# ShinYwings/SingleHDR-tf2

Hardware: AMD Instinct MI355X
Metric: HDR images/sec (512x512) end-to-end inference, deq+lin+hal (higher is better)
Workload: dtype f32

## Files before the change

### include/shdr.h

```cpp
#ifndef SHDR_H_
#define SHDR_H_

#include <stdint.h>

#ifdef __cplusplus
extern "C" {
#endif

void shdr_config_reload(void);

#define SHDR_OK          0
#define SHDR_E_SHAPE    (-1)
#define SHDR_E_ALIGN    (-2)
#define SHDR_E_ARCH     (-3)
#define SHDR_E_LAUNCH   (-4)
#define SHDR_E_NULL     (-5)

#define SHDR_ACT_NONE   0
#define SHDR_ACT_RELU   1
#define SHDR_ACT_LRELU  2
#define SHDR_ACT_TANH   3

#define SHDR_ALGO_AUTO    0
#define SHDR_ALGO_MFMA    1
#define SHDR_ALGO_DIRECT  2
#define SHDR_ALGO_MFMA_REG 3
#define SHDR_ALGO_MFMA_F16  4
#define SHDR_ALGO_MFMA_BF16 5
#define SHDR_ALGO_AUTO_F16  6
#define SHDR_ALGO_AUTO_BF16 7
#define SHDR_ALGO_AUTO_EXACT 8

const char* shdr_last_error(void);
const char* shdr_version(void);

uint32_t shdr_crc32c(const void* data, uint64_t n, uint32_t crc);

int shdr_same_pad(int in_size, int k, int stride, int* out_size, int* pad_before);

typedef struct shdr_conv2d_desc {
  int32_t N, H, W;
  int32_t C1, C2;
  int32_t Cout, KH, KW;
  int32_t stride;
  int32_t pad_t, pad_l;
  int32_t Ho, Wo;
  float   x2_scale;
  int32_t act1, act2;
  int32_t res_cstride;
  int32_t y_cstride;
  int32_t algo;
  int32_t cout_valid;
  int64_t w_batch_stride;
  int32_t y_pix_stride, y_off_h, y_off_w, y_H, y_W;
  int32_t prologue;
  int32_t pool;
} shdr_conv2d_desc;
enum { SHDR_POOL_MAX = 0, SHDR_POOL_AVG = 1 };
enum { SHDR_PROLOGUE_NONE = 0, SHDR_PROLOGUE_BILINEAR2X = 1,
       SHDR_PROLOGUE_RANGE_SCALE = 2 };

int shdr_conv2d_fwd_f32(const shdr_conv2d_desc* d,
                        const float* x1, const float* x2, const float* w,
                        const float* bias, const float* scale, const float* shift,
                        const float* residual, float* y, void* stream);

int shdr_conv2d_fwd_yrange_f32(const shdr_conv2d_desc* d,
                               const float* x1, const float* x2, const float* w,
                               const float* bias, const float* scale, const float* shift,
                               const float* residual, float* y, float* y_range, void* stream);

enum {
  SHDR_PLAN_DIRECT = 0,
  SHDR_PLAN_MFMA = 1,
  SHDR_PLAN_WINOGRAD_FUSED = 2,
  SHDR_PLAN_WINOGRAD_PLANES = 3,
  SHDR_PLAN_X3 = 4,
  SHDR_PLAN_X3N = 5
};
int shdr_conv2d_plan_f32(const shdr_conv2d_desc* d, int has_residual);
int64_t shdr_conv2d_prepared_filter_elems_f32(const shdr_conv2d_desc* d, int has_residual);
int shdr_conv2d_filter_is_plain_f32(const shdr_conv2d_desc* d, int has_residual);
int shdr_conv2d_prepare_filter_f32(const shdr_conv2d_desc* d, int has_residual, const float* w, float* prepared, void* stream);
int64_t shdr_conv2d_workspace_bytes_f32(const shdr_conv2d_desc* d, int has_residual);
int shdr_conv2d_fwd_prepared_f32(const shdr_conv2d_desc* d, const float* x1, const float* x2, const float* prepared,
                                 const float* bias, const float* scale, const float* shift, const float* residual, float* y,
                                 float* y_pool, void* workspace, void* stream);
int shdr_conv2d_fwd_prepared_ranged_f32(const shdr_conv2d_desc* d, const float* x1, const float* x2, const float* prepared,
                                        const float* bias, const float* scale, const float* shift, const float* residual, float* y,
                                        float* y_pool, void* workspace, const float* x1_range, const float* x2_range, float* y_range,
                                        void* stream);
int shdr_conv2d_projected_ok_f32(const shdr_conv2d_desc* d);
int shdr_conv2d_fwd_prepared_projected_f32(const shdr_conv2d_desc* d, const float* x1, const float* x2, const float* prepared,
                                           const float* bias, const float* scale, const float* shift, const float* proj, float* y_proj,
                                           float* y, float* y_pool, void* workspace, const float* x1_range, const float* x2_range,
                                           float* y_range, void* stream);

int shdr_conv2d_up2_lowres_ok_f32(const shdr_conv2d_desc* d);
int64_t shdr_conv2d_up2_lowres_filter_elems_f32(const shdr_conv2d_desc* d);
int shdr_conv2d_up2_lowres_prepare_filter_f32(const shdr_conv2d_desc* d, const float* w, float* prepared, void* stream);
int64_t shdr_conv2d_up2_lowres_workspace_bytes_f32(const shdr_conv2d_desc* d);
int shdr_conv2d_fwd_up2_lowres_f32(const shdr_conv2d_desc* d, const float* x, const float* prepared, const float* bias,
                                   const float* scale, const float* shift, float* y, void* workspace, const float* x_range,
                                   float* y_range, void* stream);

int shdr_conv2d_up2_fused_ok_f32(const shdr_conv2d_desc* d);
int shdr_conv2d_up2_narrow_enabled(void);
int64_t shdr_conv2d_up2_fused_filter_elems_f32(const shdr_conv2d_desc* d);
int shdr_conv2d_up2_fused_prepare_filter_f32(const shdr_conv2d_desc* d, const float* w, float* prepared, void* stream);
int shdr_conv2d_fwd_up2_fused_f32(const shdr_conv2d_desc* d, const float* x, const float* prepared, const float* bias,
                                  const float* scale, const float* shift, const float* proj, float* y_proj, float* y,
                                  const float* x_range, float* y_range, void* stream);

int shdr_conv2d_wgrad_f32(const shdr_conv2d_desc* d, const float* x, int which, const float* dz,
                          float* dw, void* stream);
int shdr_filter_transform_f32(const float* w, float* wt, int KH, int KW, int Cin, int Cout,
                              int c_begin, int c_count, float scale, void* stream);
int64_t shdr_conv2d_dgrad_workspace_bytes_f32(const shdr_conv2d_desc* d, int which);
int shdr_conv2d_dgrad_f32(const shdr_conv2d_desc* d, int which, const float* dz, const float* w, float* dx, void* workspace,
                          void* stream);
int shdr_conv2d_dgrad_tracks_range_f32(const shdr_conv2d_desc* d, int which);
int shdr_conv2d_dgrad_ranged_f32(const shdr_conv2d_desc* d, int which, const float* dz, const float* w, float* dx, void* workspace,
                                 const float* dz_range, float* dx_range, void* stream);
enum { SHDR_OP_CONV2D_FWD = 0, SHDR_OP_CONV2D_DGRAD = 1, SHDR_OP_CONV2D_WGRAD_WINOGRAD = 2, SHDR_OP_BATCHNORM = 3,
       SHDR_OP_ACT_BWD_BIAS = 4  };
#define SHDR_BN_MAX_BLOCKS 1024
int64_t shdr_workspace_bytes(int op, const shdr_conv2d_desc* d, int arg);
int shdr_bias_grad_f32(const float* dz, float* db, int64_t npix, int C, void* stream);

int shdr_soft_hist_fwd_f32(const float* x, float* y, int64_t npix, int C, int B, void* stream);
int shdr_soft_hist_bwd_f32(const float* x, const float* dy, float* dx, int64_t npix, int C, int B, void* stream);

int shdr_lin_frontend_fwd_f32(const float* img, float* y, int N, int H, int W,
                              int y_channels, void* stream);

int shdr_avgpool2_fwd_f32(const float* x, float* y, int N, int H, int W, int C, void* stream);
int shdr_maxpool2_fwd_f32(const float* x, float* y, int N, int H, int W, int C, void* stream);
int shdr_maxpool3s2_fwd_f32(const float* x, float* y, int N, int H, int W, int C, void* stream);
int shdr_resize2x_fwd_f32(const float* x, float* y, int N, int H, int W, int C, void* stream);
int shdr_gap_fwd_f32(const float* x, float* y, int N, int HW, int C, void* stream);

int shdr_invcrf_decode_fwd_f32(const float* feat, const float* wfc, const float* bfc,
                               const float* table, float* out, int B, int F, int K,
                               void* stream);
int shdr_increase_fwd_f32(const float* rf, float* out, int B, int K, void* stream);
int shdr_apply_rf_fwd_f32(const float* x, const float* rf, float* y, int B,
                          int64_t n_per_batch, int K, void* stream);

int shdr_clip_fwd_f32(const float* x, float* y, int64_t n, float lo, float hi, void* stream);
int shdr_vgg_preprocess_fwd_f32(const float* x, float* y, int64_t npix, int out_channels,
                                void* stream);
int shdr_reverse3_fwd_f32(const float* x, float* y, int64_t npix, void* stream);
int shdr_alpha_blend_fwd_f32(const float* b, const float* hal, float* a, float* alpha_out,
                             int64_t npix, float thr, void* stream);
int shdr_pack3_fwd_f32(const float* s0, const float* s1, const float* s2, const float* s3,
                       int nsrc, float* y, int out_channels, int64_t npix, void* stream);
int shdr_pad_channels_f32(const float* x, float* y, int64_t npix, int Cin, int Cout, void* stream);
// ... 389 lines not shown
```

### singlehdr-tf2_amd/_lib.py

```python
import ctypes
import os

_HERE = os.path.dirname(os.path.abspath(__file__))
LIB_PATH = os.environ.get("SHDR_LIB") or os.path.join(_HERE, "libshdr.so")

c_int = ctypes.c_int
c_i64 = ctypes.c_int64
c_f32 = ctypes.c_float
c_ptr = ctypes.c_void_p


class ConvDesc(ctypes.Structure):
    _fields_ = [("N", ctypes.c_int32), ("H", ctypes.c_int32), ("W", ctypes.c_int32),
                ("C1", ctypes.c_int32), ("C2", ctypes.c_int32),
                ("Cout", ctypes.c_int32), ("KH", ctypes.c_int32), ("KW", ctypes.c_int32),
                ("stride", ctypes.c_int32), ("pad_t", ctypes.c_int32), ("pad_l", ctypes.c_int32),
                ("Ho", ctypes.c_int32), ("Wo", ctypes.c_int32),
                ("x2_scale", ctypes.c_float),
                ("act1", ctypes.c_int32), ("act2", ctypes.c_int32),
                ("res_cstride", ctypes.c_int32), ("y_cstride", ctypes.c_int32),
                ("algo", ctypes.c_int32), ("cout_valid", ctypes.c_int32),
                ("w_batch_stride", ctypes.c_int64),
                ("y_pix_stride", ctypes.c_int32), ("y_off_h", ctypes.c_int32), ("y_off_w", ctypes.c_int32),
                ("y_H", ctypes.c_int32), ("y_W", ctypes.c_int32),
# ... 9 lines not shown
    "shdr_resize_cubic_f32": (c_int, [c_ptr, c_ptr, c_int, c_int, c_int, c_int, c_int, c_int, c_ptr]),
    "shdr_pad_symmetric_f32": (c_int, [c_ptr, c_ptr, c_int, c_int, c_int, c_int, c_int, c_ptr]),
    "shdr_rgbe_encode_f32": (c_int, [c_ptr, c_ptr, c_i64, c_int, c_ptr]),
    "shdr_rgbe_rle_encode": (c_i64, [c_ptr, c_int, c_int, c_ptr, c_i64]),
    "shdr_rgbe_rle_decode": (c_i64, [c_ptr, c_i64, c_int, c_int, c_ptr]),
    "shdr_rgbe_rle_encode_batch_sizes": (c_int, [c_ptr, c_int, ctypes.POINTER(c_i64), ctypes.POINTER(c_i64)]),
    "shdr_rgbe_rle_encode_batch": (c_int, [c_ptr, c_ptr, c_ptr, c_int, c_ptr, c_i64, c_ptr, c_ptr, c_ptr]),
    "shdr_rgbe_rle_encode_batch_timed": (c_int, [c_ptr, c_ptr, c_ptr, c_int, c_ptr, c_i64, c_ptr, c_ptr, c_ptr, c_ptr]),
    "shdr_hdr_load_resize_f32": (c_int, [c_ptr, c_ptr, c_int, c_int, c_int, c_int, c_ptr]),
    "shdr_hdr_window_means_f32": (c_int, [c_ptr, c_ptr, c_ptr, c_int, c_ptr, c_ptr, c_ptr]),
    "shdr_hdr_patch_sample_f32": (c_int, [c_ptr] * 5 + [c_int] * 4 + [c_ptr, c_ptr]),
    "shdr_exr_rle_decode": (c_i64, [c_ptr, c_i64, c_ptr, c_i64]),
    "shdr_exr_unpredict_u8": (c_int, [c_ptr, c_ptr, c_i64, c_ptr, c_ptr, c_int, c_ptr]),
    "shdr_exr_load_resize_f32": (c_int, [c_ptr, c_i64, c_ptr, c_int, c_int, c_i64, c_ptr, c_ptr, c_int, c_int, c_ptr, c_int, c_int,
                                         c_int, c_ptr]),
    "shdr_deflate_huffman_host": (c_i64, [c_ptr, c_i64, c_ptr, c_i64]),
    "shdr_deflate_huffman_lengths_host": (c_int, [c_ptr, c_i64, c_ptr]),
    "shdr_deflate_huffman_batch_sizes": (c_int, [c_ptr, c_int, c_int, ctypes.POINTER(c_i64), ctypes.POINTER(c_i64)]),
    "shdr_deflate_huffman_batch": (c_int, [c_ptr, c_ptr, c_ptr, c_ptr, c_int, c_int, c_ptr, c_i64, c_ptr, c_ptr, c_ptr, c_ptr, c_ptr]),
    "shdr_deflate_lz_host": (c_i64, [c_ptr, c_i64, c_ptr, c_i64]),
    "shdr_deflate_lz_parse_host": (c_int, [c_ptr, c_i64, c_ptr]),
    "shdr_deflate_lz_batch_sizes": (c_int, [c_ptr, c_int, c_int, ctypes.POINTER(c_i64), ctypes.POINTER(c_i64)]),
    "shdr_deflate_lz_batch": (c_int, [c_ptr, c_ptr, c_ptr, c_ptr, c_int, c_int, c_ptr, c_i64, c_ptr, c_ptr, c_ptr, c_ptr, c_ptr]),
    "shdr_inflate_host": (c_i64, [c_ptr, c_i64, c_ptr, c_i64, ctypes.POINTER(c_int)]),
    "shdr_inflate_batch_sizes": (c_int, [c_ptr, c_ptr, c_int, ctypes.POINTER(c_i64), ctypes.POINTER(c_i64)]),
    "shdr_piz_decode_host": (c_i64, [c_ptr, c_i64, c_int, c_int, c_ptr, c_int, c_ptr, c_i64, ctypes.POINTER(c_int)]),
    "shdr_piz_batch_sizes": (c_int, [c_ptr, c_ptr, c_ptr, c_ptr, c_int, c_int, c_int] + [ctypes.POINTER(c_i64)] * 3),
    "shdr_piz_batch": (c_int, [c_ptr, c_i64, c_ptr, c_ptr, c_ptr, c_i64, c_ptr, c_ptr, c_ptr, c_ptr, c_ptr, c_ptr, c_ptr, c_int, c_int, c_int,
                               c_ptr, c_i64, c_ptr, c_ptr, c_ptr, c_ptr, c_ptr]),
    "shdr_inflate_batch": (c_int, [c_ptr, c_i64, c_ptr, c_ptr, c_ptr, c_i64, c_ptr, c_ptr, c_ptr, c_int, c_ptr, c_ptr, c_ptr, c_ptr]),
    "shdr_exr_pack_sizes": (c_int, [c_ptr, c_int, c_int, c_int, ctypes.POINTER(c_i64), ctypes.POINTER(c_i64), c_ptr, c_ptr]),
    "shdr_exr_pack_f32": (c_int, [c_ptr, c_ptr, c_int, c_int, c_int, c_int, c_int, c_ptr, c_ptr, c_ptr, c_ptr, c_ptr]),
    "shdr_exr_finish_chunks": (c_int, [c_ptr, c_ptr, c_ptr, c_ptr, c_ptr, c_int, c_i64, c_int, c_ptr]),
    "shdr_philox4x32_10": (c_int, [c_ptr, c_ptr, c_ptr]),
    "shdr_camera_expose_f32": (c_int, [c_ptr, c_ptr, c_ptr, c_ptr, c_int, c_int, c_int, ctypes.c_uint64, c_ptr]),
    "shdr_jpeg_round_trip_f32": (c_int, [c_ptr] * 6 + [c_int, c_int, c_int, c_ptr]),
    "shdr_flip_rot90_f32": (c_int, [c_ptr, c_ptr, c_ptr, c_ptr, c_int, c_int, c_int, c_f32, c_ptr]),
    "shdr_pair_patch_stats": (c_int, [c_ptr, c_ptr, c_i64, c_ptr, c_ptr, c_int, c_ptr, c_ptr, c_int, c_int, c_ptr, c_ptr, c_ptr]),
    "shdr_pair_patch_gather_f32": (c_int, [c_ptr, c_ptr, c_i64, c_ptr, c_ptr, c_int, c_ptr, c_ptr, c_int, c_ptr, c_ptr, c_ptr, c_int,
                                           c_int, c_ptr, c_ptr, c_ptr]),
    "shdr_conv2d_winograd_fused_f32": (c_int, [c_ptr] * 6 + [c_int] * 7 + [c_ptr]),
    "shdr_conv2d_winograd_fused2_f32": (c_int, [c_ptr] * 8 + [c_int] * 8 + [c_ptr]),
    "shdr_conv2d_winograd_fused_up2_f32": (c_int, [c_ptr] * 6 + [c_int] * 7 + [c_ptr]),
    "shdr_conv2d_x3_ok_f32": (c_int, [ctypes.POINTER(ConvDesc)]),
    "shdr_conv2d_x3_filter_elems_f32": (c_i64, [ctypes.POINTER(ConvDesc)]),
    "shdr_conv2d_x3_prepare_filter_f32": (c_int, [ctypes.POINTER(ConvDesc), c_ptr, c_ptr, c_ptr]),
    "shdr_conv2d_fwd_x3_f32": (c_int, [ctypes.POINTER(ConvDesc)] + [c_ptr] * 9),
    "shdr_conv2d_fwd_x3_ranged_f32": (c_int, [ctypes.POINTER(ConvDesc)] + [c_ptr] * 12),
    "shdr_absmax_f32": (c_int, [c_ptr, c_i64, c_ptr, c_ptr]),
    "shdr_x3_split_planes_f32": (c_int, [c_ptr, c_i64, c_ptr, c_ptr, c_ptr, c_ptr]),
    "shdr_conv2d_wgrad_x3_ok_f32": (c_int, [ctypes.POINTER(ConvDesc), c_int]),
    "shdr_conv2d_wgrad_x3_f32": (c_int, [ctypes.POINTER(ConvDesc), c_ptr, c_ptr, c_int, c_ptr, c_ptr, c_ptr, c_ptr, c_ptr, c_ptr]),
    "shdr_config_reload": (None, []),
    "shdr_conv2d_x3_input_absmax_f32": (c_int, [c_ptr, c_i64, c_ptr, c_ptr]),
    "shdr_conv2d_x3n_ok_f32": (c_int, [ctypes.POINTER(ConvDesc)]),
    "shdr_conv2d_x3n_filter_elems_f32": (c_i64, [ctypes.POINTER(ConvDesc)]),
    "shdr_conv2d_x3n_prepare_filter_f32": (c_int, [ctypes.POINTER(ConvDesc), c_ptr, c_ptr, c_ptr]),
    "shdr_conv2d_fwd_x3n_f32": (c_int, [ctypes.POINTER(ConvDesc)] + [c_ptr] * 10),
    "shdr_conv2d_fwd_x3n_ranged_f32": (c_int, [ctypes.POINTER(ConvDesc)] + [c_ptr] * 13),
    "shdr_act_bwd_bias_f32": (c_int, [c_ptr, c_ptr, c_ptr, c_ptr, c_ptr, c_i64, c_int, c_int, c_ptr]),
    "shdr_winograd_filter_packed_f32": (c_int, [c_ptr, c_ptr, c_int, c_int, c_ptr]),
    "shdr_conv2d_wgrad_winograd_f32": (c_int, [c_ptr] * 4 + [c_int] * 7 + [c_f32, c_ptr]),
    "shdr_crc32c": (ctypes.c_uint32, [c_ptr, ctypes.c_uint64, ctypes.c_uint32]),
    "shdr_same_pad": (c_int, [c_int, c_int, c_int, ctypes.POINTER(c_int), ctypes.POINTER(c_int)]),
    "shdr_conv2d_fwd_f32": (c_int, [ctypes.POINTER(ConvDesc)] + [c_ptr] * 9),
    "shdr_conv2d_fwd_yrange_f32": (c_int, [ctypes.POINTER(ConvDesc)] + [c_ptr] * 10),
    "shdr_conv2d_plan_f32": (c_int, [ctypes.POINTER(ConvDesc), c_int]),
    "shdr_conv2d_prepared_filter_elems_f32": (c_i64, [ctypes.POINTER(ConvDesc), c_int]),
    "shdr_conv2d_filter_is_plain_f32": (c_int, [ctypes.POINTER(ConvDesc), c_int]),
    "shdr_conv2d_prepare_filter_f32": (c_int, [ctypes.POINTER(ConvDesc), c_int, c_ptr, c_ptr, c_ptr]),
    "shdr_conv2d_workspace_bytes_f32": (c_i64, [ctypes.POINTER(ConvDesc), c_int]),
    "shdr_conv2d_fwd_prepared_f32": (c_int, [ctypes.POINTER(ConvDesc)] + [c_ptr] * 11),
    "shdr_conv2d_fwd_prepared_ranged_f32": (c_int, [ctypes.POINTER(ConvDesc)] + [c_ptr] * 14),
    "shdr_conv2d_projected_ok_f32": (c_int, [ctypes.POINTER(ConvDesc)]),
    "shdr_conv2d_fwd_prepared_projected_f32": (c_int, [ctypes.POINTER(ConvDesc)] + [c_ptr] * 15),
    "shdr_conv2d_up2_lowres_ok_f32": (c_int, [ctypes.POINTER(ConvDesc)]),
    "shdr_conv2d_up2_lowres_filter_elems_f32": (c_i64, [ctypes.POINTER(ConvDesc)]),
    "shdr_conv2d_up2_lowres_prepare_filter_f32": (c_int, [ctypes.POINTER(ConvDesc), c_ptr, c_ptr, c_ptr]),
    "shdr_conv2d_up2_lowres_workspace_bytes_f32": (c_i64, [ctypes.POINTER(ConvDesc)]),
    "shdr_conv2d_fwd_up2_lowres_f32": (c_int, [ctypes.POINTER(ConvDesc)] + [c_ptr] * 10),
    "shdr_conv2d_up2_fused_ok_f32": (c_int, [ctypes.POINTER(ConvDesc)]),
    "shdr_conv2d_up2_narrow_enabled": (c_int, []),
    "shdr_conv2d_up2_fused_filter_elems_f32": (c_i64, [ctypes.POINTER(ConvDesc)]),
    "shdr_conv2d_up2_fused_prepare_filter_f32": (c_int, [ctypes.POINTER(ConvDesc), c_ptr, c_ptr, c_ptr]),
    "shdr_conv2d_fwd_up2_fused_f32": (c_int, [ctypes.POINTER(ConvDesc)] + [c_ptr] * 11),
    "shdr_conv2d_fwd_x3_projected_f32": (c_int, [ctypes.POINTER(ConvDesc)] + [c_ptr] * 14),
    "shdr_conv2d_fwd_x3_residual_f32": (c_int, [ctypes.POINTER(ConvDesc)] + [c_ptr] * 12),
    "shdr_conv2d_dgrad_workspace_bytes_f32": (c_i64, [ctypes.POINTER(ConvDesc), c_int]),
    "shdr_conv2d_dgrad_f32": (c_int, [ctypes.POINTER(ConvDesc), c_int, c_ptr, c_ptr, c_ptr, c_ptr, c_ptr]),
    "shdr_conv2d_dgrad_tracks_range_f32": (c_int, [ctypes.POINTER(ConvDesc), c_int]),
    "shdr_conv2d_dgrad_ranged_f32": (c_int, [ctypes.POINTER(ConvDesc), c_int, c_ptr, c_ptr, c_ptr, c_ptr, c_ptr, c_ptr, c_ptr]),
    "shdr_workspace_bytes": (c_i64, [c_int, ctypes.POINTER(ConvDesc), c_int]),
    "shdr_soft_hist_bwd_f32": (c_int, [c_ptr, c_ptr, c_ptr, c_i64, c_int, c_int, c_ptr]),
    "shdr_conv2d_wgrad_f32": (c_int, [ctypes.POINTER(ConvDesc), c_ptr, c_int, c_ptr, c_ptr, c_ptr]),
    "shdr_filter_transform_f32": (c_int, [c_ptr, c_ptr, c_int, c_int, c_int, c_int, c_int, c_int, c_f32, c_ptr]),
    "shdr_bias_grad_f32": (c_int, [c_ptr, c_ptr, c_i64, c_int, c_ptr]),
    "shdr_soft_hist_fwd_f32": (c_int, [c_ptr, c_ptr, c_i64, c_int, c_int, c_ptr]),
    "shdr_lin_frontend_fwd_f32": (c_int, [c_ptr, c_ptr, c_int, c_int, c_int, c_int, c_ptr]),
    "shdr_avgpool2_fwd_f32": (c_int, [c_ptr, c_ptr, c_int, c_int, c_int, c_int, c_ptr]),
    "shdr_maxpool2_fwd_f32": (c_int, [c_ptr, c_ptr, c_int, c_int, c_int, c_int, c_ptr]),
    "shdr_maxpool3s2_fwd_f32": (c_int, [c_ptr, c_ptr, c_int, c_int, c_int, c_int, c_ptr]),
    "shdr_resize2x_fwd_f32": (c_int, [c_ptr, c_ptr, c_int, c_int, c_int, c_int, c_ptr]),
    "shdr_gap_fwd_f32": (c_int, [c_ptr, c_ptr, c_int, c_int, c_int, c_ptr]),
    "shdr_invcrf_decode_fwd_f32": (c_int, [c_ptr] * 5 + [c_int, c_int, c_int, c_ptr]),
    "shdr_increase_fwd_f32": (c_int, [c_ptr, c_ptr, c_int, c_int, c_ptr]),
    "shdr_apply_rf_fwd_f32": (c_int, [c_ptr, c_ptr, c_ptr, c_int, c_i64, c_int, c_ptr]),
    "shdr_clip_fwd_f32": (c_int, [c_ptr, c_ptr, c_i64, c_f32, c_f32, c_ptr]),
    "shdr_vgg_preprocess_fwd_f32": (c_int, [c_ptr, c_ptr, c_i64, c_int, c_ptr]),
    "shdr_reverse3_fwd_f32": (c_int, [c_ptr, c_ptr, c_i64, c_ptr]),
    "shdr_alpha_blend_fwd_f32": (c_int, [c_ptr, c_ptr, c_ptr, c_ptr, c_i64, c_f32, c_ptr]),
    "shdr_pack3_fwd_f32": (c_int, [c_ptr] * 4 + [c_int, c_ptr, c_int, c_i64, c_ptr]),
    "shdr_logc_fwd_f32": (c_int, [c_ptr, c_ptr, c_i64, c_ptr]),
    "shdr_affine_act_f32": (c_int, [c_ptr] * 5 + [c_i64, c_int, c_int, c_ptr]),
    "shdr_pad_channels_f32": (c_int, [c_ptr, c_ptr, c_i64, c_int, c_int, c_ptr]),
    "shdr_act_bwd_f32": (c_int, [c_ptr, c_ptr, c_ptr, c_i64, c_int, c_ptr]),
    "shdr_clip_bwd_f32": (c_int, [c_ptr, c_ptr, c_ptr, c_i64, c_f32, c_f32, c_ptr]),
    "shdr_add_f32": (c_int, [c_ptr, c_ptr, c_ptr, c_i64, c_ptr]),
    "shdr_add_ranged_f32": (c_int, [c_ptr, c_ptr, c_ptr, c_i64, c_ptr, c_ptr]),
    "shdr_avgpool2_bwd_f32": (c_int, [c_ptr, c_ptr, c_int, c_int, c_int, c_int, c_ptr]),
    "shdr_maxpool2_bwd_f32": (c_int, [c_ptr, c_ptr, c_ptr, c_int, c_int, c_int, c_int, c_ptr]),
    "shdr_maxpool3s2_bwd_f32": (c_int, [c_ptr, c_ptr, c_ptr, c_ptr, c_int, c_int, c_int, c_int, c_ptr]),
    "shdr_resize2x_bwd_f32": (c_int, [c_ptr, c_ptr, c_int, c_int, c_int, c_int, c_ptr]),
    "shdr_resize2x_bwd_ranged_f32": (c_int, [c_ptr, c_ptr, c_int, c_int, c_int, c_int, c_ptr, c_ptr]),
    "shdr_gap_bwd_f32": (c_int, [c_ptr, c_ptr, c_int, c_int, c_int, c_ptr]),
    "shdr_upsample_zero2_f32": (c_int, [c_ptr, c_ptr, c_int, c_int, c_int, c_int, c_ptr]),
    "shdr_bn_stats_f32": (c_int, [c_ptr] * 6 + [c_i64, c_int, c_f32, c_ptr]),
    "shdr_bn_train_apply_f32": (c_int, [c_ptr] * 6 + [c_i64, c_int, c_f32, c_int, c_ptr]),
    "shdr_bn_train_apply_ranged_f32": (c_int, [c_ptr] * 6 + [c_i64, c_int, c_f32, c_int, c_ptr, c_ptr]),
    "shdr_bn_bwd_f32": (c_int, [c_ptr] * 10 + [c_i64, c_int, c_f32, c_ptr]),
    "shdr_bn_bwd_ranged_f32": (c_int, [c_ptr] * 10 + [c_i64, c_int, c_f32, c_ptr, c_ptr]),
    "shdr_invcrf_decode_bwd_f32": (c_int, [c_ptr] * 7 + [c_int, c_int, c_int, c_ptr]),
    "shdr_increase_bwd_f32": (c_int, [c_ptr, c_ptr, c_ptr, c_int, c_int, c_ptr]),
    "shdr_apply_rf_bwd_f32": (c_int, [c_ptr] * 5 + [c_int, c_i64, c_int, c_ptr]),
    "shdr_diff_loss_f32": (c_int, [c_ptr, c_ptr, c_ptr, c_int, c_i64, c_int, c_ptr]),
# ... 91 lines not shown
```

### singlehdr-tf2_amd/_ops.py

```python
import collections
import ctypes
import math

import numpy as np
import torch

try:
    from . import _lib
except ImportError:
    import _lib

AUTOGRAD = None


def _needs_grad(*tensors):
    return AUTOGRAD is not None and torch.is_grad_enabled() and any(
        isinstance(t, torch.Tensor) and t.requires_grad for t in tensors)


WINOGRAD = True


ACT_NONE, ACT_RELU, ACT_LRELU, ACT_TANH = 0, 1, 2, 3
ALGO_AUTO, ALGO_MFMA, ALGO_DIRECT, ALGO_MFMA_REG = 0, 1, 2, 3
PROLOGUE_NONE, PROLOGUE_BILINEAR2X = 0, 1
POOL_MAX, POOL_AVG = 0, 1
ALGO_MFMA_F16, ALGO_MFMA_BF16, ALGO_AUTO_F16, ALGO_AUTO_BF16 = 4, 5, 6, 7
ALGO_AUTO_EXACT = 8
EXACT_FP32 = False


def _auto(algo):
    return ALGO_AUTO_EXACT if (algo == ALGO_AUTO and EXACT_FP32) else algo

PRECISION = "fp32"
_AUTO_ALGO = {"fp32": ALGO_AUTO, "fp16": ALGO_AUTO, "fp16op": ALGO_AUTO_F16, "bf16": ALGO_AUTO_BF16}


def native_fp16():
    return PRECISION == "fp16"


class precision:

    def __init__(self, name):
        if name not in _AUTO_ALGO:
            raise ValueError("precision must be one of %s" % sorted(_AUTO_ALGO))
        self._name = name

    def __enter__(self):
        global PRECISION
        self._prev, PRECISION = PRECISION, self._name
        return self

    def __exit__(self, *exc):
# ... 179 lines not shown


def up2_narrow_enabled():
    return bool(_lib.load().shdr_conv2d_up2_narrow_enabled())


def _up2_layer(form, x, w, bias, act1, scale, shift, act2):
    lib = _lib.load()
    x, w_var = _d(x), w
    w = _d(w)
    if x.dim() != 4 or w.dim() != 4 or tuple(w.shape[:2]) != (3, 3) or w.shape[2] != x.shape[3]:
        return None
    n, h, wd, c1 = x.shape
    cout = w.shape[3]
    d = _lib.ConvDesc()
    d.N, d.H, d.W, d.C1, d.C2 = n, 2 * h, 2 * wd, c1, 0
    d.Cout, d.KH, d.KW, d.stride = cout, 3, 3, 1
    d.cout_valid, d.y_cstride = cout, cout
    d.pad_t, d.pad_l, d.Ho, d.Wo = 1, 1, 2 * h, 2 * wd
    d.x2_scale = 1.0
    d.act1, d.act2 = act1, act2
    d.algo = ALGO_AUTO
    d.prologue = PROLOGUE_BILINEAR2X
    if not int(getattr(lib, "shdr_conv2d_up2_%s_ok_f32" % form)(ctypes.byref(d))):
        return None
    _chk(x, "x")
    _chk(w, "w")
    for t, nm in ((bias, "bias"), (scale, "scale"), (shift, "shift")):
        if t is not None and (_chk(_d(t), nm).numel() != cout):
            raise ValueError("conv2d_up2: %s must have %d elements" % (nm, cout))
    persistent = _is_persistent(w_var)
    nprep = int(getattr(lib, "shdr_conv2d_up2_%s_filter_elems_f32" % form)(ctypes.byref(d)))
    key = ("up2_" + form, c1, cout, nprep)
    prepared = _filter_cache_get(w_var, "_shdr_packed", key) if persistent else None
    if prepared is None:
        prepared = torch.empty(nprep, device=w.device, dtype=torch.float32)
        name = "shdr_conv2d_up2_%s_prepare_filter_f32" % form
        _lib.check(getattr(lib, name)(ctypes.byref(d), _ptr(w), _ptr(prepared), _stream()), name)
        if persistent:
            _filter_cache_put(w_var, "_shdr_packed", key, prepared)
    return d, x, prepared


def _conv2d_up2_lowres(x, w, bias, act1, scale, shift, act2):
    layer = _up2_layer("lowres", x, w, bias, act1, scale, shift, act2)
    if layer is None:
        return None
    lib = _lib.load()
    x_in = x
    d, x, prepared = layer
    xr = _range_of(x_in)
    if xr is None:
        RANGE_MISSES[(tuple(x.shape), None, tuple(_d(w).shape))] += 1
    ws = torch.empty(int(lib.shdr_conv2d_up2_lowres_workspace_bytes_f32(ctypes.byref(d))), device=x.device, dtype=torch.uint8)
    out = torch.empty((d.N, d.H, d.W, d.Cout), device=x.device, dtype=torch.float32)
    yr = _new_slot(x.device)
    rc = lib.shdr_conv2d_fwd_up2_lowres_f32(ctypes.byref(d), _ptr(x), _ptr(prepared), _ptr(_d(bias)), _ptr(_d(scale)), _ptr(_d(shift)),
                                            _ptr(out), _ptr(ws), _ptr(xr), _ptr(yr), _stream())
    _lib.check(rc, "shdr_conv2d_fwd_up2_lowres_f32")
    return _set_range(out, yr)


def _conv2d_up2_fused(x, w, bias, act1, scale, shift, act2, proj=None, want_y=None):
    if proj is not None and _d(w).shape[-1] != 64:
        return None
    layer = _up2_layer("fused", x, w, bias, act1, scale, shift, act2)
    if layer is None:
        return None
    lib = _lib.load()
    x_in = x
    d, x, prepared = layer
    if proj is not None:
        proj = _chk(_d(proj), "proj")
        if tuple(proj.shape) != (3, d.Cout):
            raise ValueError("conv2d_up2: proj must be [3, %d]" % d.Cout)
    if want_y is None:
        want_y = proj is None
    xr = _range_of(x_in)
    if xr is None:
        RANGE_MISSES[(tuple(x.shape), None, tuple(_d(w).shape))] += 1
        xr = _new_slot(x.device)
        _lib.check(lib.shdr_absmax_f32(_ptr(x), x.numel(), _ptr(xr), _stream()), "shdr_absmax_f32")
    out = torch.empty((d.N, d.H, d.W, d.Cout), device=x.device, dtype=torch.float32) if want_y else None
    yj = torch.empty((d.N, d.H, d.W, 3), device=x.device, dtype=torch.float32) if proj is not None else None
    yr = _new_slot(x.device) if want_y else None
    rc = lib.shdr_conv2d_fwd_up2_fused_f32(ctypes.byref(d), _ptr(x), _ptr(prepared), _ptr(_d(bias)), _ptr(_d(scale)), _ptr(_d(shift)),
                                           _ptr(proj), _ptr(yj), _ptr(out), _ptr(xr), _ptr(yr), _stream())
    _lib.check(rc, "shdr_conv2d_fwd_up2_fused_f32")
    if proj is not None:
        PROJECTED_LAUNCHES[0] += 1
    if want_y:
        _set_range(out, yr)
    return out if proj is None else ((yj, out) if want_y else yj)


def _conv2d_raw(x, w, bias, stride, x2, x2_scale, act1, scale, shift, residual, act2, algo, out, cout_valid, pad, out_hw,
                w_batch_stride, pool, prologue=0, proj=None):
    lib = _lib.load()
    x_in, x2_in = x, x2
    x = _chk(_d(x), "x")
    w_var = w
    w = _chk(_d(w), "w")
    n, h, wd, c1 = x.shape
    if prologue == PROLOGUE_BILINEAR2X:
        h, wd = 2 * h, 2 * wd
    kh, kw, cin, cout_gemm = w.shape
    cout = cout_gemm if cout_valid is None else int(cout_valid)
    c2 = 0
    if x2 is not None:
        x2 = _chk(_d(x2), "x2")
        if x2.shape[:3] != x.shape[:3]:
            raise ValueError("conv2d: x2 spatial shape %s != x %s" % (tuple(x2.shape), tuple(x.shape)))
# ... 1945 lines not shown
```

### singlehdr-tf2_amd/build.py

```python
import os
import shutil
import subprocess
import sys

HERE = os.path.dirname(os.path.abspath(__file__))
CSRC = os.path.join(HERE, "csrc")
INCLUDE = os.path.normpath(os.path.join(HERE, "..", "include"))
OBJ_DIR = os.path.join(HERE, "build")
LIB = os.path.join(HERE, "libshdr.so")

SOURCES = {
    "api.cpp": [],
    "conv.hip": [],
    "conv_plan.hip": [],
    "conv_x3.hip": [],
    "conv_x3n.hip": [],
    "conv_f16.hip": [],
    "conv_f16_patch.hip": [],
    "conv_f16_w3.hip": [],
    "wgrad_x3.hip": [],
    "wgrad_f16.hip": [],
    "wgrad_f16_alltaps.hip": [],
    "elem_f16.hip": ["-ffp-contract=off"],
    "wgrad.hip": [],
    "wgrad_winograd.hip": [],
    "bwd.hip": [],
    "finetune.hip": [],
    "winograd.hip": [],
    "winograd_fused.hip": [],
    "frontend.hip": ["-ffp-contract=off"],
    "pool.hip": [],
    "up2_lowres.hip": [],
    "up2_fused.hip": [],
    "crf.hip": [],
    "glue.hip": [],
    "imageio.hip": [],
    "hdr_rle.hip": [],
    "metrics.hip": [],
    "camera.hip": ["-ffp-contract=off"],
    "dataset.hip": ["-ffp-contract=off"],
    "exr.hip": ["-ffp-contract=off"],
    "exr_write.hip": ["-ffp-contract=off"],
    "deflate.hip": [],
    "deflate_lz.hip": [],
    "inflate.hip": [],
    "piz.hip": [],
    "hdr_real.hip": ["-ffp-contract=off"],
    "jpeg.hip": ["-ffp-contract=off"],
    "jpeg_scan.hip": [],
}
COMMON = ["-O3", "-std=c++17", "-fPIC", "--offload-arch=gfx950", "-I" + INCLUDE, "-I" + CSRC,
          "-Wall", "-Wno-unused-function"]


def _hipcc():
    for cand in (os.environ.get("HIPCC"), shutil.which("hipcc"), "/opt/rocm/bin/hipcc"):
        if cand and os.path.exists(cand):
            return cand
    raise RuntimeError("hipcc not found (set HIPCC)")


def _stale(target, deps):
    if not os.path.exists(target):
        return True
    t = os.path.getmtime(target)
    return any(os.path.getmtime(d) > t for d in deps)


def build(force=False, verbose=True):
    hipcc = _hipcc()
    os.makedirs(OBJ_DIR, exist_ok=True)
    headers = [os.path.join(CSRC, "shdr_internal.h"), os.path.join(CSRC, "linear_resize.h"), os.path.join(CSRC, "jpeg_int.h"), os.path.join(CSRC, "deflate_huffman.h"),
               os.path.join(CSRC, "deflate_lz.h"), os.path.join(CSRC, "deflate_batch.h"),
               os.path.join(CSRC, "inflate.h"), os.path.join(CSRC, "piz.h"), os.path.join(CSRC, "jpeg_scan.h"),
               os.path.join(CSRC, "exr_half.h"), os.path.join(INCLUDE, "shdr.h"), __file__]
    objs = []
    procs = []
    for src, extra in SOURCES.items():
        s = os.path.join(CSRC, src)
        o = os.path.join(OBJ_DIR, os.path.splitext(src)[0] + ".o")
        objs.append(o)
        if force or _stale(o, [s] + headers):
            cmd = [hipcc] + COMMON + extra + ["-x", "hip", "-c", s, "-o", o]
            if verbose:
                print(" ".join(cmd), flush=True)
            procs.append((src, subprocess.Popen(cmd)))
    for src, p in procs:
        if p.wait() != 0:
            raise RuntimeError("hipcc failed on " + src)
    if force or procs or _stale(LIB, objs):
        cmd = [hipcc, "-shared", "-fPIC", "--offload-arch=gfx950", "-o", LIB] + objs
        if verbose:
            print(" ".join(cmd), flush=True)
        subprocess.check_call(cmd)
    return LIB


if __name__ == "__main__":
    print(build(force="--force" in sys.argv))
```

### singlehdr-tf2_amd/csrc/api.cpp

```cpp
#include <stdarg.h>
#include <stdio.h>
#include <string.h>

#include "shdr_internal.h"

namespace shdr {
static thread_local char g_last_error[512] = "";

void set_error(const char* fmt, ...) {
  va_list ap;
  va_start(ap, fmt);
  vsnprintf(g_last_error, sizeof(g_last_error), fmt, ap);
  va_end(ap);
}
}

namespace shdr {
int g_env_epoch = 0;
}
extern "C" void shdr_config_reload(void) { __atomic_add_fetch(&shdr::g_env_epoch, 1, __ATOMIC_ACQ_REL); }

extern "C" const char* shdr_last_error(void) { return shdr::g_last_error; }
extern "C" const char* shdr_version(void) { return "libshdr 0.1 gfx950"; }

namespace {
struct Crc32cTable {
  uint32_t t[8][256];
  Crc32cTable() {
    for (uint32_t i = 0; i < 256; ++i) {
      uint32_t c = i;
      for (int k = 0; k < 8; ++k) c = (c & 1) ? (c >> 1) ^ 0x82F63B78u : c >> 1;
      t[0][i] = c;
    }
    for (uint32_t i = 0; i < 256; ++i)
      for (int s = 1; s < 8; ++s) t[s][i] = (t[s - 1][i] >> 8) ^ t[0][t[s - 1][i] & 0xff];
  }
};
}

extern "C" uint32_t shdr_crc32c(const void* data, uint64_t n, uint32_t crc) {
  static const Crc32cTable tab;
  const unsigned char* p = static_cast<const unsigned char*>(data);
  uint32_t c = ~crc;
  while (n >= 8) {
    const uint32_t lo = c ^ ((uint32_t)p[0] | (uint32_t)p[1] << 8 | (uint32_t)p[2] << 16 | (uint32_t)p[3] << 24);
    c = tab.t[7][lo & 0xff] ^ tab.t[6][(lo >> 8) & 0xff] ^ tab.t[5][(lo >> 16) & 0xff] ^ tab.t[4][lo >> 24] ^
        tab.t[3][p[4]] ^ tab.t[2][p[5]] ^ tab.t[1][p[6]] ^ tab.t[0][p[7]];
    p += 8;
    n -= 8;
  }
  while (n--) c = tab.t[0][(c ^ *p++) & 0xff] ^ (c >> 8);
  return ~c;
}

namespace {
int64_t rle_component(const uint8_t* data, int n, uint8_t* out) {
  constexpr int kMinRun = 4;
  int64_t w = 0;
  int cur = 0;
  while (cur < n) {
    int run_start = cur, run_len = 0, prev_len = 0;
    while (run_len < kMinRun && run_start < n) {
      run_start += run_len;
      prev_len = run_len;
      run_len = 1;
      while (run_start + run_len < n && run_len < 127 && data[4 * run_start] == data[4 * (run_start + run_len)]) ++run_len;
    }
    if (prev_len > 1 && prev_len == run_start - cur) {
      out[w++] = (uint8_t)(128 + prev_len);
      out[w++] = data[4 * cur];
      cur = run_start;
    }
    while (cur < run_start) {
// ... 124 lines not shown
```

### singlehdr-tf2_amd/csrc/conv_x3.hip

```cpp
#include <hip/hip_fp16.h>
#include <stdlib.h>

#include <type_traits>

#include "shdr_internal.h"

namespace {

using f32x4 = __attribute__((ext_vector_type(4))) float;
using f16x8 = __attribute__((ext_vector_type(8))) _Float16;
using f16x4 = __attribute__((ext_vector_type(4))) _Float16;
using u32x4 = __attribute__((ext_vector_type(4))) unsigned;

constexpr int X3_HEADER_FLOATS = 16;
constexpr int BN = 64, NT = 4, MT = 4;
constexpr int IMG_HALVES = BN * 32;
constexpr int UNIT_HALVES = 2 * IMG_HALVES;
constexpr int LRW = 10, LRPIX = LRW * LRW;
constexpr int LRJ = (LRPIX * 8 + 255) / 256;
template <int KH, int KW>
struct X3G {
  static constexpr int PH = 16 + KH - 1, PWID = 16 + KW - 1, PPIX = PH * PWID;
  static constexpr int PJ = (PPIX * 8 + 255) / 256;
  static constexpr int PATCH_HALVES = PPIX * 32;
  static constexpr int LDS_BYTES = (2 * PATCH_HALVES + 2 * UNIT_HALVES) * 2;
  static constexpr int LDS_BYTES_UP = LDS_BYTES + LRPIX * 32 * 4;
  static constexpr int RANGE_BYTES = 16;
};

struct X3Args {
  const float* x1;
  const float* x2;
  const _Float16* wp;
  const float* hdr;
  const float* bias;
  const float* scale;
  const float* shift;
  float* y;
  float* yp;
  const float* res;
  int res_cs;
  int N, H, W, C1, C2, Cout, tiles_x, tiles_y, nblk_m, nblk_n, act1, act2;
  int Hl, Wl;
  int Hin, Win;
  int in_s, bh, bw;
  int pool_avg;
  const unsigned* xr1;
  const unsigned* xr2;
  unsigned* yr;
  int nphase;
  int pth[4], ptw[4], pbh[4], pbw[4];
  const _Float16* pwp[4];
  const float* proj;
  float* yproj;
};

__device__ __forceinline__ void x3_range_scale(const unsigned* r1, const unsigned* r2, float& xs, float& ixs) {
  xs = 1.0f;
  ixs = 1.0f;
  unsigned b = r1 ? *r1 : 0u;
  if (r2) {
    const unsigned b2 = *r2;
    b = b2 > b ? b2 : b;
  }
  if (b != 0u && b < 0x7f800000u) {
    int ex;
    frexpf(__uint_as_float(b), &ex);
    int T = 11 - ex;
    T = T < -126 ? -126 : (T > 126 ? 126 : T);
    xs = ldexpf(1.0f, T);
    ixs = ldexpf(1.0f, -T);
  }
}
__device__ __forceinline__ void x3_split4(const f32x4 v, float xs, unsigned (&h)[2], unsigned (&l)[2]) {
  const float k2048 = 2048.0f;
#pragma unroll
  for (int p = 0; p < 2; ++p) {
    float t0, t1;
    asm("v_fma_mixlo_f16 %0, %1, %2, 0" : "=v"(h[p]) : "v"(v[2 * p]), "s"(xs));
    asm("v_fma_mixhi_f16 %0, %1, %2, 0" : "+v"(h[p]) : "v"(v[2 * p + 1]), "s"(xs));
    asm("v_fma_mix_f32 %0, %1, %2, -%3 op_sel_hi:[0,0,1]" : "=v"(t0) : "v"(v[2 * p]), "s"(xs), "v"(h[p]));
    asm("v_fma_mix_f32 %0, %1, %2, -%3 op_sel:[0,0,1] op_sel_hi:[0,0,1]" : "=v"(t1) : "v"(v[2 * p + 1]), "s"(xs), "v"(h[p]));
    asm("v_fma_mixlo_f16 %0, %1, %2, 0" : "=v"(l[p]) : "v"(t0), "s"(k2048));
    asm("v_fma_mixhi_f16 %0, %1, %2, 0" : "+v"(l[p]) : "v"(t1), "s"(k2048));
  }
}
template <int NW = 4>
__device__ __forceinline__ void x3_range_out(unsigned* slot, float m, int lane, int wave, unsigned seen, unsigned* lds) {
#pragma unroll
  for (int off = 32; off > 0; off >>= 1) m = fmaxf(m, __shfl_xor(m, off, 64));
  if (lane == 0) lds[wave] = __float_as_uint(m);
  asm volatile("s_waitcnt lgkmcnt(0)\n\ts_barrier" ::: "memory");
  if (threadIdx.x == 0) {
    const unsigned b01 = lds[0] > lds[1] ? lds[0] : lds[1], b23 = lds[2] > lds[3] ? lds[2] : lds[3];
    unsigned b = b01 > b23 ? b01 : b23;
    if (NW == 8) {
      const unsigned b45 = lds[4] > lds[5] ? lds[4] : lds[5], b67 = lds[6] > lds[7] ? lds[6] : lds[7];
      const unsigned b47 = b45 > b67 ? b45 : b67;
      b = b47 > b ? b47 : b;
    }
#ifndef SHDR_ABL_NO_RANGE_ATOMIC
    if (b > seen) atomicMax(slot, b);
#endif
  }
}

template <int NW, bool PROJ>
// ... 51 lines not shown
#pragma unroll
          for (int j = 0; j < 3; ++j) {
            const f32x4 q = *reinterpret_cast<const f32x4*>(a.proj + j * 64 + cl);
            pj[r][j] += v[r][0] * q[0] + v[r][1] * q[1] + v[r][2] * q[2] + v[r][3] * q[3];
          }
        }
#ifndef SHDR_ABL_NO_YM
        if (a.yr && oh + r < a.H) ym = fmaxf(fmaxf(fmaxf(fmaxf(ym, fabsf(v[r][0])), fabsf(v[r][1])), fabsf(v[r][2])), fabsf(v[r][3]));
#endif
      }
      if (a.yp) {
        f32x4 m;
#pragma unroll
        for (int e = 0; e < 4; ++e) {
          if (a.pool_avg) {
            const float t = v[0][e] + __shfl_xor(v[0][e], 1, 64), b = v[1][e] + __shfl_xor(v[1][e], 1, 64);
            m[e] = 0.25f * (t + b);
          } else {
            m[e] = fmaxf(v[0][e], v[1][e]);
            m[e] = fmaxf(m[e], __shfl_xor(m[e], 1, 64));
          }
        }
        if (!(pc & 1) && ow < a.W && n0 + cl < a.Cout)
          *reinterpret_cast<f32x4*>(a.yp + ((size_t)(img * (a.H >> 1) + (oh >> 1)) * (a.W >> 1) + (ow >> 1)) * a.Cout + n0 + cl) = m;
      }
    }
    if (PROJ && a.proj) {
#pragma unroll
      for (int r = 0; r < 2; ++r) {
#pragma unroll
        for (int j = 0; j < 3; ++j) {
          float t = pj[r][j];
          t += __shfl_xor(t, 16, 64);
          t += __shfl_xor(t, 32, 64);
          pj[r][j] = t;
        }
        if (fg == 0 && oh + r < a.H && ow < a.W) {
          float* o = a.yproj + ((size_t)(img * a.H + oh + r) * a.W + ow) * 3;
          o[0] = pj[r][0]; o[1] = pj[r][1]; o[2] = pj[r][2];
        }
      }
    }
  }
#ifndef SHDR_ABL_NO_TAIL
  if (a.yr)
    x3_range_out<NW>(a.yr, ow < a.W ? ym : 0.0f, lane, wave, yr_seen, range_lds);
#endif
}

__device__ __forceinline__ int xcd_remap(int bid, int nwg) {
  const int q = nwg >> 3, r = nwg & 7, xcd = bid & 7, idx = bid >> 3;
  return (xcd < r ? xcd * (q + 1) : r * (q + 1) + (xcd - r) * q) + idx;
}
__host__ __device__ inline int f4(int row) { return (-(row >> 2)) & 3; }
__host__ __device__ inline int sx(int col) { return ((col >> 2) & 1) * 2; }
__device__ __forceinline__ int pcol(int fi) { return fi < 4 ? fi : (fi >= 12 ? fi - 8 : fi + 4); }

template <bool UP, int KH, int KW, bool MP = false, int LOOK = 1>
__global__ __launch_bounds__(256, 2) void conv_x3_kernel(const X3Args a) {
  using G = X3G<KH, KW>;
  constexpr int PWID = G::PWID, PPIX = G::PPIX, PJ = G::PJ, PATCH_HALVES = G::PATCH_HALVES, NTAPS = KH * KW;
  static_assert(!UP || (KH == 3 && KW == 3), "the up-sampling prologue belongs to the 3 x 3 stride-1 form");
  static_assert(!MP || (!UP && KH == 4 && KW == 4), "the phase loop is built on the 4 x 4 patch geometry");
  static_assert(LOOK >= 1 && LOOK <= 2 && LOOK <= KW, "filter look-ahead: 1 or 2 taps");
  extern __shared__ __attribute__((aligned(16))) _Float16 xsm[];
#define patch_h (xsm)
#define patch_l (xsm + PATCH_HALVES)
#define filt (xsm + 2 * PATCH_HALVES)
#define lrs (reinterpret_cast<float*>(xsm + 2 * PATCH_HALVES + 2 * UNIT_HALVES))

  const int tid = threadIdx.x, lane = tid & 63;
  const int wave = __builtin_amdgcn_readfirstlane(tid >> 6);
  const int L = xcd_remap(blockIdx.x, a.nblk_m * a.nblk_n);
  const int pn = L % a.nblk_n;
  int pm = L / a.nblk_n;
  const int tx = pm % a.tiles_x;
  pm /= a.tiles_x;
  const int ty = pm % a.tiles_y;
  const int img = pm / a.tiles_y;
  const int n0 = pn * BN, oh0 = ty * 16, ow0 = tx * 16;

  int ppix[PJ];
  int pdst[PJ];
  int pcnt = 0;
  auto patch_geometry = [&](int bh, int bw) __attribute__((always_inline)) {
    pcnt = 0;
#pragma unroll
    for (int j = 0; j < (UP ? 0 : PJ); ++j) {
      const int p = tid + 256 * j;
      const int pix = p >> 3, q = p & 7;
      const int py = pix / PWID, px = pix - py * PWID;
      const int ih = a.in_s * (oh0 + py) + bh, iw = a.in_s * (ow0 + px) + bw;
      const bool ok = pix < PPIX && (unsigned)ih < (unsigned)a.Hin && (unsigned)iw < (unsigned)a.Win;
      ppix[j] = ok ? (img * a.Hin + ih) * a.Win + iw : -1;
      pdst[j] = pix < PPIX ? pix * 32 + 8 * ((q >> 1) ^ sx(px)) + 4 * (q & 1) : -1;
      pcnt += __ballot(ppix[j] >= 0) != 0ull;
    }
  };
  if (!MP) patch_geometry(a.bh, a.bw);
  if (!MP && !UP) pcnt = __builtin_amdgcn_readfirstlane(pcnt);
  int lpix[LRJ];
  if (UP) {
#pragma unroll
    for (int j = 0; j < LRJ; ++j) {
      const int p = tid + 256 * j;
      const int pix = p >> 3;
      const int ly = pix / LRW, lx = pix - ly * LRW;
      const int r = (oh0 >> 1) - 1 + ly, c = (ow0 >> 1) - 1 + lx;
      lpix[j] = (pix < LRPIX && (unsigned)r < (unsigned)a.Hl && (unsigned)c < (unsigned)a.Wl) ? (img * a.Hl + r) * a.Wl + c : -1;
      pcnt += __ballot(lpix[j] >= 0) != 0ull;
    }
    pcnt = __builtin_amdgcn_readfirstlane(pcnt);
  }
  const int nch1 = a.C1 >> 5, nch = (a.C1 + a.C2) >> 5;
  int nunits = nch * NTAPS;
  constexpr int DEPTH = (NTAPS == 1 && !UP && !MP) ? 2 : 1;
  using Set0 = std::integral_constant<int, 0>;
  using Set1 = std::integral_constant<int, DEPTH - 1>;
  f32x4 pr_sets[DEPTH][PJ];
#define pr (pr_sets[0])
  auto zero_patch = [&](auto setc) __attribute__((always_inline)) {
    constexpr int S = decltype(setc)::value;
#pragma unroll
    for (int j = 0; j < (UP ? LRJ : PJ); ++j) pr_sets[S][j] = (f32x4){0.f, 0.f, 0.f, 0.f};
#pragma unroll
    for (int j = 0; j < (UP ? LRJ : PJ); ++j) asm volatile("" : "+v"(pr_sets[S][j]));
// ... 210 lines not shown
    } else {
#pragma unroll
      for (int kh = 0; kh < KH; ++kh) {
#pragma unroll
        for (int kw = 0; kw < KW; ++kw) X3_TAP(kh == 0)
      }
      asm volatile("s_waitcnt vmcnt(0)" : "+v"(fr[0][0]), "+v"(fr[0][1]) : : "memory");
#pragma unroll
      for (int j = 0; j < FJ; ++j) fr[NFR - 1][j] = fr[0][j];
    }
#undef X3_TAP
#undef X3_SLOT
    if (c + 1 < nch) {
      if (UP) {
        park_lr();
        __syncthreads();
      } else {
        __syncthreads();
      }
      store_patch(nxt);
    }
  };
#pragma unroll 1
  for (int c = 0; c < nch; c += DEPTH) {
    chunk(c, Set0{}, Set1{});
    if (DEPTH == 2 && c + 1 < nch) chunk(c + 1, Set1{}, Set0{});
  }
  }
#undef pr
#undef X3_WAIT_VM

  x3_tile_epilogue<4, true>(a, acc, img, oh0 + wave * MT, ow0 + pc, pc, fg, n0, ixs, lane, wave,
                            reinterpret_cast<unsigned*>(reinterpret_cast<char*>(xsm) + (UP ? G::LDS_BYTES_UP : G::LDS_BYTES)));
}

#undef patch_h
#undef patch_l
#undef filt
#undef lrs

constexpr int X1_BP = 128;
template <int NS>
__global__ __launch_bounds__(256, 2) void conv_x3_1x1_kernel(const X3Args a) {
  constexpr int MT1 = 2 * NS, BP = X1_BP;
  constexpr int PJ1 = BP * 8 / 256;
  constexpr int IMG = BP * 32;
  static_assert(NS * (BP / (MT1 * 16)) == 4, "four waves: NS cout slices x pixel groups");
  __shared__ __attribute__((aligned(16))) _Float16 x1sm[2 * 2 * IMG];
  __shared__ unsigned x1rw[4];

  const int tid = threadIdx.x, lane = tid & 63;
  const int wave = __builtin_amdgcn_readfirstlane(tid >> 6);
  const int slice = wave % NS, grp = wave / NS;
  const int L = xcd_remap(blockIdx.x, a.nblk_m * a.nblk_n);
  const int pn = L % a.nblk_n, pm = L / a.nblk_n;
  const int P0 = pm * BP, Ptot = a.N * a.H * a.W;

  int ppix[PJ1];
  const int pdst = (tid >> 3) * 32 + 8 * (((tid & 7) >> 1) ^ sx((tid >> 3) & 15)) + 4 * (tid & 1);
#pragma unroll
  for (int j = 0; j < PJ1; ++j) {
    const int P = P0 + (tid >> 3) + 32 * j;
    ppix[j] = -1;
    if (P < Ptot) {
      const int ow = P % a.W, t = P / a.W;
      const int oh = t % a.H, img = t / a.H;
      const int ih = a.in_s * oh + a.bh, iw = a.in_s * ow + a.bw;
      if ((unsigned)ih < (unsigned)a.Hin && (unsigned)iw < (unsigned)a.Win) ppix[j] = (img * a.Hin + ih) * a.Win + iw;
    }
  }
  const int nch1 = a.C1 >> 5, nch = (a.C1 + a.C2) >> 5;
  using Set0 = std::integral_constant<int, 0>;
  using Set1 = std::integral_constant<int, 1>;
  f32x4 pr_sets[2][PJ1];
  auto load_patch = [&](int c, auto setc) __attribute__((always_inline)) {
    constexpr int S = decltype(setc)::value;
    const bool second = c >= nch1;
    const float* src = second ? a.x2 : a.x1;
    const int Cs = second ? a.C2 : a.C1;
    const int c0 = (second ? c - nch1 : c) << 5;
#pragma unroll
    for (int j = 0; j < PJ1; ++j) {
      pr_sets[S][j] = (f32x4){0.f, 0.f, 0.f, 0.f};
      if (ppix[j] >= 0) pr_sets[S][j] = *reinterpret_cast<const f32x4*>(src + (size_t)(unsigned)ppix[j] * (unsigned)Cs + c0 + 4 * (tid & 7));
    }
  };
  float xs = 1.0f, ixs = 1.0f;
  auto store_patch = [&](int buf, auto setc) __attribute__((always_inline)) {
    constexpr int S = decltype(setc)::value;
#pragma unroll
    for (int j = 0; j < PJ1; ++j) {
      unsigned h[2], l[2];
      x3_split4(pr_sets[S][j], xs, h, l);
      *reinterpret_cast<uint2*>(x1sm + buf * 2 * IMG + pdst + 1024 * j) = make_uint2(h[0], h[1]);
      *reinterpret_cast<uint2*>(x1sm + buf * 2 * IMG + IMG + pdst + 1024 * j) = make_uint2(l[0], l[1]);
    }
  };
  const int fi = lane & 15, fg = lane >> 4;
  const _Float16* wsl = a.wp + (size_t)(pn * NS + slice) * nch * UNIT_HALVES + fi * 32 + 8 * fg;
  f16x8 f0h[2], f0l[2], f1h[2], f1l[2];
  auto load_w = [&](int c, int half, f16x8 (&h)[2], f16x8 (&l)[2]) __attribute__((always_inline)) {
    const _Float16* g = wsl + (size_t)c * UNIT_HALVES + half * 2 * 16 * 32;
#pragma unroll
    for (int k = 0; k < 2; ++k) {
      h[k] = *reinterpret_cast<const f16x8*>(g + k * 16 * 32);
      l[k] = *reinterpret_cast<const f16x8*>(g + IMG_HALVES + k * 16 * 32);
    }
// ... 79 lines not shown
#pragma unroll
      for (int e = 0; e < EB; ++e)
#pragma unroll
        for (int ni = 0; ni < NT; ++ni) {
          const int P = Pw + 16 * (m0 + e);
          res_r[e][ni] = P < Ptot ? *reinterpret_cast<const f32x4*>(a.res + (size_t)P * a.res_cs + ep0 + ni * 16 + 4 * fg) : (f32x4){0.f, 0.f, 0.f, 0.f};
        }
    }
#pragma unroll
    for (int e = 0; e < EB; ++e) {
      const int P = Pw + 16 * (m0 + e);
      if (P0 + grp * MT1 * 16 + 16 * (m0 + e) >= Ptot) continue;
#pragma unroll
      for (int ni = 0; ni < NT; ++ni) {
        f32x4 v = acc[m0 + e][ni] * inv_s;
        asm("" : "+v"(v));
        v += bias_r[ni];
        shdr::act_apply4<0>(v, a.act1);
        if (a.scale) v = v * scale_r[ni] + shift_r[ni];
        if (a.res) v += res_r[e][ni];
        shdr::act_apply4<0>(v, a.act2);
        if (P < Ptot) {
          *reinterpret_cast<f32x4*>(a.y + (size_t)P * a.Cout + ep0 + ni * 16 + 4 * fg) = v;
          if (a.yr) ym = fmaxf(fmaxf(fmaxf(fmaxf(ym, fabsf(v[0])), fabsf(v[1])), fabsf(v[2])), fabsf(v[3]));
        }
      }
    }
  }
  if (a.yr) x3_range_out(a.yr, ym, lane, wave, yr_seen, x1rw);
}

constexpr int XW_THREADS = 512, XW_BN = 128;
constexpr long XW_UP_MIN_COUT = 128;
struct XWG {
  using G = X3G<3, 3>;
  static constexpr int PJ = (G::PPIX * 8 + XW_THREADS - 1) / XW_THREADS;
  static constexpr int RANGE_BYTES = 32;
  static constexpr int LR_BYTES = LRPIX * 32 * 4;
  static constexpr int LDS_BYTES = (2 * 2 * G::PATCH_HALVES + 2 * 2 * UNIT_HALVES) * 2;
};
template <bool UP>
__global__ __launch_bounds__(XW_THREADS, 2) void conv_x3_wide_kernel(const X3Args a) {
  using G = X3G<3, 3>;
  constexpr int KH = 3, KW = 3, PWID = G::PWID, PPIX = G::PPIX, PJ = XWG::PJ, PATCH_HALVES = G::PATCH_HALVES, NTAPS = 9;
  static_assert((PJ - 1) * XW_THREADS < PPIX * 8 && PJ == 6, "every piece but the last is inside the patch for every thread");
  extern __shared__ __attribute__((aligned(16))) _Float16 xsm[];
#define patch_buf(B) (xsm + (B) * 2 * PATCH_HALVES)
#define filt (xsm + 4 * PATCH_HALVES)
#define lrs (reinterpret_cast<float*>(xsm + 4 * PATCH_HALVES + 4 * UNIT_HALVES))

  const int tid = threadIdx.x, lane = tid & 63;
  const int wave = __builtin_amdgcn_readfirstlane(tid >> 6);
  const int slice = wave >> 2, wq = wave & 3;
  const int L = xcd_remap(blockIdx.x, a.nblk_m * a.nblk_n);
  const int pn = L % a.nblk_n;
  int pm = L / a.nblk_n;
  const int tx = pm % a.tiles_x;
  pm /= a.tiles_x;
  const int ty = pm % a.tiles_y;
  const int img = pm / a.tiles_y;
  const int n0 = pn * XW_BN + slice * BN, oh0 = ty * 16, ow0 = tx * 16;

  constexpr int PL = UP ? (LRPIX * 8 + XW_THREADS - 1) / XW_THREADS : PJ;
  constexpr int T0 = UP ? 4 : 3;
  int ppix[PL], pdst[PJ];
  int pcnt = 0;
  if (UP) {
#pragma unroll
    for (int j = 0; j < PL; ++j) {
      const int p = tid + XW_THREADS * j;
      const int pix = p >> 3;
      const int ly = pix / LRW, lx = pix - ly * LRW;
      const int r = (oh0 >> 1) - 1 + ly, c = (ow0 >> 1) - 1 + lx;
      ppix[j] = (pix < LRPIX && (unsigned)r < (unsigned)a.Hl && (unsigned)c < (unsigned)a.Wl) ? (img * a.Hl + r) * a.Wl + c : -1;
      pcnt += __ballot(ppix[j] >= 0) != 0ull;
    }
  }
#pragma unroll
  for (int j = 0; j < (UP ? 0 : PJ); ++j) {
    const int p = tid + XW_THREADS * j;
    const int pix = p >> 3, q = p & 7;
    const int py = pix / PWID, px = pix - py * PWID;
    const int ih = oh0 + py + a.bh, iw = ow0 + px + a.bw;
    const bool ok = pix < PPIX && (unsigned)ih < (unsigned)a.Hin && (unsigned)iw < (unsigned)a.Win;
    ppix[j] = ok ? (img * a.Hin + ih) * a.Win + iw : -1;
    pdst[j] = pix < PPIX ? pix * 32 + 8 * ((q >> 1) ^ sx(px)) + 4 * (q & 1) : -1;
    pcnt += __ballot(ppix[j] >= 0) != 0ull;
  }
  pcnt = __builtin_amdgcn_readfirstlane(pcnt);
  const int nch1 = a.C1 >> 5, nch = (a.C1 + a.C2) >> 5;
  const int nunits = nch * NTAPS;
  f32x4 pr[PL];
  auto zero_patch = [&]() __attribute__((always_inline)) {
#pragma unroll
    for (int j = 0; j < PL; ++j) pr[j] = (f32x4){0.f, 0.f, 0.f, 0.f};
#pragma unroll
    for (int j = 0; j < PL; ++j) asm volatile("" : "+v"(pr[j]));
  };
  auto load_patch = [&](int c, bool zeroed) __attribute__((always_inline)) {
    if (UP) {
#pragma unroll
      for (int j = 0; j < PL; ++j) {
        const int q = (tid + XW_THREADS * j) & 7;
        if (!zeroed) pr[j] = (f32x4){0.f, 0.f, 0.f, 0.f};
        if (ppix[j] >= 0) pr[j] = *reinterpret_cast<const f32x4*>(a.x1 + (size_t)(unsigned)ppix[j] * (unsigned)a.C1 + (c << 5) + 4 * q);
      }
      return;
// ... 419 lines not shown
  const int64_t n4 = shdr::aligned16(x) ? n / 4 : 0;
  if (n4 > 0) {
    int grid = shdr::stream_grid(n4);
    if (grid > 1024) grid = 1024;
    hipLaunchKernelGGL(x3_absmax_big_kernel, dim3(grid), dim3(256), 0, st, x, (long)n4, slot);
  }
  if (n - 4 * n4 > 0) hipLaunchKernelGGL(x3_absmax_kernel, dim3(n4 > 0 ? 1 : (shdr::stream_grid(n) < 64 ? shdr::stream_grid(n) : 64)), dim3(256), 0, st, x + 4 * n4, (long)(n - 4 * n4), slot);
  return shdr::check_launch("absmax");
}

extern "C" int shdr_conv2d_x3_input_absmax_f32(const float* x, int64_t n, float* prepared, void* stream) {
  SHDR_REQUIRE(x && prepared, SHDR_E_NULL, "conv2d_x3_input_absmax: null pointer");
  SHDR_REQUIRE(n > 0 && n % 4 == 0 && shdr::aligned16(x), SHDR_E_SHAPE, "conv2d_x3_input_absmax: n must be a positive multiple of 4, x 16-byte aligned");
  return shdr_absmax_f32(x, n, prepared + 2, stream);
}

static int x3_forward(const shdr_conv2d_desc* d, const float* x1, const float* x2, const float* prepared, const float* bias,
                      const float* scale, const float* shift, const float* residual, float* y, float* y_pool, const float* proj, float* y_proj,
                      const float* x1_range, const float* x2_range, float* y_range, void* stream) {
  SHDR_REQUIRE(d && x1 && prepared && (y || y_pool || y_proj), SHDR_E_NULL, "conv2d_x3: null desc/x1/filter or no output");
  SHDR_REQUIRE((proj == nullptr) == (y_proj == nullptr), SHDR_E_NULL, "conv2d_x3: proj and y_proj come together");
  SHDR_REQUIRE(!proj || (d->Cout == 64 && d->stride == 1 && shdr::aligned16(proj)), SHDR_E_SHAPE,
               "conv2d_x3: the projected output takes a stride-1 layer with 64 output channels (one cout slice per block) and a 16-byte aligned map");
  SHDR_REQUIRE(!y_pool || (d->Ho % 2 == 0 && d->Wo % 2 == 0 && shdr::aligned16(y_pool)), SHDR_E_SHAPE, "conv2d_x3: the fused 2x2 max-pool needs even Ho, Wo");
  const bool up = d->prologue == SHDR_PROLOGUE_BILINEAR2X, rs = d->prologue == SHDR_PROLOGUE_RANGE_SCALE;
  SHDR_REQUIRE(d->prologue == SHDR_PROLOGUE_NONE || rs || (up && d->stride == 1 && d->C2 == 0 && d->H % 2 == 0 && d->W % 2 == 0), SHDR_E_SHAPE,
               "conv2d_x3: the bilinear 2x prologue takes a stride-1 layer, one source and even (up-sampled) H, W");
  SHDR_REQUIRE(shdr_conv2d_x3_ok_f32(d), SHDR_E_SHAPE, "conv2d_x3: layer shape not taken by this kernel");
  SHDR_REQUIRE((d->C2 == 0) == (x2 == nullptr), SHDR_E_NULL, "conv2d_x3: x2 must be given iff C2 > 0");
  SHDR_REQUIRE((scale == nullptr) == (shift == nullptr), SHDR_E_NULL, "conv2d_x3: scale and shift come together");
  SHDR_REQUIRE(shdr::aligned16(x1) && (!x2 || shdr::aligned16(x2)) && shdr::aligned16(prepared) && (!y || shdr::aligned16(y)) &&
                   (!bias || shdr::aligned16(bias)) && (!scale || (shdr::aligned16(scale) && shdr::aligned16(shift))),
               SHDR_E_ALIGN, "conv2d_x3: tensors must be 16-byte aligned");
  SHDR_REQUIRE(!x2 || ((x1_range == nullptr) == (x2_range == nullptr)), SHDR_E_NULL, "conv2d_x3: give the range of both sources or of neither");
  X3Args a{};
  a.x1 = x1; a.x2 = x2 ? x2 : x1;
  a.bias = bias; a.scale = scale; a.shift = shift; a.y = y; a.yp = y_pool;
  a.pool_avg = d->pool == SHDR_POOL_AVG;
  a.N = d->N; a.H = d->Ho; a.W = d->Wo; a.C1 = d->C1; a.C2 = d->C2; a.Cout = d->Cout;
  a.Hin = d->H; a.Win = d->W;
  a.Hl = d->H / 2; a.Wl = d->W / 2;
  a.tiles_x = (a.W + 15) / 16;
  a.tiles_y = (a.H + 15) / 16;
  a.nblk_m = a.N * a.tiles_x * a.tiles_y;
  a.nblk_n = (a.Cout + 63) / 64;
  a.act1 = d->act1; a.act2 = d->act2;
  a.xr1 = reinterpret_cast<const unsigned*>(x1_range);
  a.xr2 = reinterpret_cast<const unsigned*>(x2 ? x2_range : nullptr);
  a.yr = reinterpret_cast<unsigned*>(y_range);
  a.proj = proj; a.yproj = y_proj;
  SHDR_REQUIRE(!residual || (d->stride == 1 && d->res_cstride >= d->Cout && d->res_cstride % 4 == 0 && shdr::aligned16(residual) && !y_pool && !proj), SHDR_E_SHAPE,
               "conv2d_x3: the residual takes a stride-1 layer, res_cstride >= Cout (a multiple of 4), a 16-byte aligned tensor, no pooled / projected output");
  a.res = residual; a.res_cs = d->res_cstride;
  hipStream_t st = reinterpret_cast<hipStream_t>(stream);
  X3Phase ph[4];
  const int n = x3_phases(d, ph);
  const int Ct = d->C1 + d->C2;
  a.hdr = prepared;
  a.wp = reinterpret_cast<const _Float16*>(prepared + X3_HEADER_FLOATS);
  if (rs && !x1_range) a.xr1 = reinterpret_cast<const unsigned*>(prepared) + 2;
  a.in_s = ph[0].step; a.bh = ph[0].bh; a.bw = ph[0].bw;
  if (n == 4) {
    const float* pk = prepared;
    a.nphase = 4;
    for (int i = 0; i < 4; ++i) {
      SHDR_REQUIRE(ph[i].th <= 4 && ph[i].tw <= 4 && ph[i].step == ph[0].step, SHDR_E_SHAPE, "conv2d_x3: unexpected phase geometry");
      a.pth[i] = ph[i].th; a.ptw[i] = ph[i].tw; a.pbh[i] = ph[i].bh; a.pbw[i] = ph[i].bw;
      a.pwp[i] = reinterpret_cast<const _Float16*>(pk + X3_HEADER_FLOATS);
      pk += x3_phase_floats(ph[i], Ct, d->Cout);
    }
    return launch_x3<false, 4, 4, true>(a, st);
  }
  if (ph[0].th == 3 && ph[0].tw == 3) {
    long wide_min_blocks = 256, wide_min_cout = up ? XW_UP_MIN_COUT : 512;
    if (const char* e = SHDR_ENV("SHDR_X3_WIDE_MIN_BLOCKS")) wide_min_blocks = atol(e);
    if (const char* e = SHDR_ENV("SHDR_X3_WIDE_MIN_COUT")) wide_min_cout = atol(e);
    const bool wide = d->stride == 1 && d->Cout % XW_BN == 0 && d->Cout >= wide_min_cout && !proj &&
                      (long)a.nblk_m * (d->Cout / XW_BN) >= wide_min_blocks && SHDR_ENV("SHDR_X3_SLICED") == nullptr;
    return wide ? (up ? launch_x3_wide<true>(a, st) : launch_x3_wide<false>(a, st)) : up ? launch_x3<true, 3, 3>(a, st) : launch_x3<false, 3, 3>(a, st);
  }
  if (ph[0].th == 1 && ph[0].tw == 1) {
    const bool wide = d->Cout % 128 == 0 && y && !y_pool && !proj && !up && SHDR_ENV("SHDR_X3_1X1_SLICED") == nullptr;
    return wide ? launch_x3_1x1(a, st) : launch_x3<false, 1, 1>(a, st);
  }
  return shdr::fail(SHDR_E_SHAPE, "conv2d_x3: no kernel for a %d x %d layer", ph[0].th, ph[0].tw);
}

extern "C" int shdr_conv2d_fwd_x3_ranged_f32(const shdr_conv2d_desc* d, const float* x1, const float* x2, const float* prepared, const float* bias,
                                             const float* scale, const float* shift, float* y, float* y_pool, const float* x1_range,
                                             const float* x2_range, float* y_range, void* stream) {
  SHDR_REQUIRE(y || y_pool, SHDR_E_NULL, "conv2d_x3: neither y nor y_pool");
  return x3_forward(d, x1, x2, prepared, bias, scale, shift, nullptr, y, y_pool, nullptr, nullptr, x1_range, x2_range, y_range, stream);
}

extern "C" int shdr_conv2d_fwd_x3_residual_f32(const shdr_conv2d_desc* d, const float* x1, const float* x2, const float* prepared, const float* bias,
                                               const float* scale, const float* shift, const float* residual, float* y, const float* x1_range,
                                               const float* x2_range, float* y_range, void* stream) {
  SHDR_REQUIRE(y, SHDR_E_NULL, "conv2d_x3: null y");
  return x3_forward(d, x1, x2, prepared, bias, scale, shift, residual, y, nullptr, nullptr, nullptr, x1_range, x2_range, y_range, stream);
}

extern "C" int shdr_conv2d_fwd_x3_projected_f32(const shdr_conv2d_desc* d, const float* x1, const float* x2, const float* prepared,
                                                const float* bias, const float* scale, const float* shift, const float* proj, float* y_proj,
                                                float* y, float* y_pool, const float* x1_range, const float* x2_range, float* y_range,
                                                void* stream) {
  SHDR_REQUIRE(proj && y_proj, SHDR_E_NULL, "conv2d_x3_projected: null proj / y_proj");
// ... 8 lines not shown
```

### singlehdr-tf2_amd/csrc/conv_x3n.hip

```cpp
#include <hip/hip_fp16.h>
#include <stdlib.h>

#include "shdr_internal.h"

namespace {

using f32x4 = __attribute__((ext_vector_type(4))) float;
using f16x8 = __attribute__((ext_vector_type(8))) _Float16;
using f16x4 = __attribute__((ext_vector_type(4))) _Float16;
typedef __attribute__((address_space(1))) const void* gptr_t;
typedef __attribute__((address_space(3))) void* lptr_t;

constexpr int XN_HEADER_FLOATS = 16;

__device__ __attribute__((aligned(16))) float g_xn_zero_page[4] = {0.f, 0.f, 0.f, 0.f};

struct X3nArgs {
  const float* x1;
  const float* x2;
  const _Float16* wp;
  const float* hdr;
  const float* bias;
  const float* scale;
  const float* shift;
  const float* res;
  float* y;
  float* yp;
  int pool_avg;
  int N, H, W, C1, tiles_x, tiles_y, ntiles, act1, act2, cout_valid, res_cs;
  const unsigned* xr1;
  const unsigned* xr2;
  unsigned* yr;
};

__device__ __forceinline__ void xn_range_scale(const unsigned* r1, const unsigned* r2, float& xs, float& ixs) {
  xs = 1.0f;
  ixs = 1.0f;
  unsigned b = r1 ? *r1 : 0u;
  if (r2) {
    const unsigned b2 = *r2;
    b = b2 > b ? b2 : b;
  }
  if (b != 0u && b < 0x7f800000u) {
    int ex;
    frexpf(__uint_as_float(b), &ex);
    int T = 11 - ex;
    T = T < -126 ? -126 : (T > 126 ? 126 : T);
    xs = ldexpf(1.0f, T);
    ixs = ldexpf(1.0f, -T);
  }
}
__device__ __forceinline__ void xn_split4(const f32x4 v, float xs, unsigned (&h)[2], unsigned (&l)[2]) {
  const float k2048 = 2048.0f;
#pragma unroll
  for (int p = 0; p < 2; ++p) {
    float t0, t1;
    asm("v_fma_mixlo_f16 %0, %1, %2, 0" : "=v"(h[p]) : "v"(v[2 * p]), "s"(xs));
    asm("v_fma_mixhi_f16 %0, %1, %2, 0" : "+v"(h[p]) : "v"(v[2 * p + 1]), "s"(xs));
    asm("v_fma_mix_f32 %0, %1, %2, -%3 op_sel_hi:[0,0,1]" : "=v"(t0) : "v"(v[2 * p]), "s"(xs), "v"(h[p]));
    asm("v_fma_mix_f32 %0, %1, %2, -%3 op_sel:[0,0,1] op_sel_hi:[0,0,1]" : "=v"(t1) : "v"(v[2 * p + 1]), "s"(xs), "v"(h[p]));
    asm("v_fma_mixlo_f16 %0, %1, %2, 0" : "=v"(l[p]) : "v"(t0), "s"(k2048));
    asm("v_fma_mixhi_f16 %0, %1, %2, 0" : "+v"(l[p]) : "v"(t1), "s"(k2048));
  }
}
__device__ __forceinline__ void xn_range_out(unsigned* slot, float m, int lane, int wave, unsigned* lds) {
#pragma unroll
  for (int off = 32; off > 0; off >>= 1) m = fmaxf(m, __shfl_xor(m, off, 64));
  if (lane == 0) lds[wave] = __float_as_uint(m);
  asm volatile("s_waitcnt lgkmcnt(0)\n\ts_barrier" ::: "memory");
  if (threadIdx.x == 0) {
    const unsigned b01 = lds[0] > lds[1] ? lds[0] : lds[1], b23 = lds[2] > lds[3] ? lds[2] : lds[3];
    const unsigned b = b01 > b23 ? b01 : b23;
#ifndef SHDR_ABL_NO_RANGE_ATOMIC
    if (b > __hip_atomic_load(slot, __ATOMIC_RELAXED, __HIP_MEMORY_SCOPE_AGENT)) atomicMax(slot, b);
#endif
  }
}

struct __attribute__((packed, aligned(4))) f32x3u { float x, y, z; };

__host__ __device__ inline int pswz(int row) { return (-(row >> 2)) & 3; }

template <int KK, int CT, int NT, bool TWO>
struct NG {
  static constexpr int TPP = 32 / CT;
// ... 38 lines not shown
#define patch_h (nsm + 2 * G::FILT_HALVES)
#define patch_l (nsm + 2 * G::FILT_HALVES + G::PATCH_HALVES)

  const int tid = threadIdx.x, lane = tid & 63;
  const int wave = __builtin_amdgcn_readfirstlane(tid >> 6);

  for (int j = wave; j < 2 * G::FINSTR; j += 4) {
    const int img = j >= G::FINSTR, jj = j - img * G::FINSTR;
    const int r = jj * 16 + (lane >> 2);
    const int co = r % G::COUT;
    const _Float16* p = a.wp + img * G::FILT_HALVES + (size_t)r * 32 + 8 * ((lane & 3) ^ pswz(co));
    __builtin_amdgcn_global_load_lds((gptr_t)p, (lptr_t)(nsm + img * G::FILT_HALVES + jj * 512), 16, 0, 0);
  }
  if (G::HALF && wave < 2) {
    static_assert(!G::HALF || G::COUT <= 32, "one DMA instruction covers 32 half rows");
    const int co = lane >> 1;
    if (co < G::COUT) {
      const int base = wave * G::FILT_HALVES + G::FULL_STEPS * G::COUT * 32;
      const _Float16* p = a.wp + base + co * 16 + 8 * ((lane & 1) ^ (pswz(co) & 1));
      __builtin_amdgcn_global_load_lds((gptr_t)p, (lptr_t)(nsm + base), 16, 0, 0);
    }
  }

  int ppy[G::PJ], ppx[G::PJ], pdst[G::PJ], pch[G::PJ];
#pragma unroll
  for (int j = 0; j < G::PJ; ++j) {
    const int piece = tid + 256 * j;
    int pix, c4, src = 0;
    if (TWO) {
      src = piece / (G::PP * 4);
      const int rem = piece - src * G::PP * 4;
      pix = rem >> 2;
      c4 = rem & 3;
    } else {
      pix = piece / (CT / 4);
      c4 = piece - pix * (CT / 4);
    }
    ppy[j] = pix / G::PW;
    ppx[j] = pix - ppy[j] * G::PW;
    const bool ok = piece < G::PIECES;
    if (TWO) {
      pdst[j] = ok ? src * G::PP * 16 + pix * 16 + 4 * c4 : -1;
      pch[j] = ok ? (src << 16) | (4 * c4) : -1;
    } else {
      const int cg = (CT == 32) ? ((c4 >> 1) ^ pswz(pix)) : (c4 >> 1);
      pdst[j] = ok ? pix * CT + 8 * cg + 4 * (c4 & 1) : -1;
      pch[j] = (ok && 4 * c4 < a.C1) ? 4 * c4 : -1;
    }
  }
  float xs = 1.0f, ixs = 1.0f;
  f32x4 pr[G::PJ];
  constexpr bool ASM_LOADS = !(CT == 8 && NT == 1);
  auto load_patch = [&](int tile) __attribute__((always_inline)) {
    int pm = tile;
    const int tx = pm % a.tiles_x;
    pm /= a.tiles_x;
    const int ty = pm % a.tiles_y;
    const int img = pm / a.tiles_y;
    const int ih0 = ty * 16 - PAD, iw0 = tx * 16 - PAD;
#pragma unroll
    for (int j = 0; j < G::PJ; ++j) {
      const int ih = ih0 + ppy[j], iw = iw0 + ppx[j];
      const bool ok = pch[j] >= 0 && (unsigned)ih < (unsigned)a.H && (unsigned)iw < (unsigned)a.W;
      const float* src = (TWO && (pch[j] >> 16)) ? a.x2 : a.x1;
      const int cs = TWO ? 16 : a.C1;
      if (!ASM_LOADS) {
        pr[j] = (f32x4){0.f, 0.f, 0.f, 0.f};
        if (ok) pr[j] = *reinterpret_cast<const f32x4*>(src + ((size_t)(img * a.H + ih) * a.W + iw) * cs + (pch[j] & 0xFFFF));
        continue;
      }
      const float* p = ok ? src + ((size_t)(img * a.H + ih) * a.W + iw) * cs + (pch[j] & 0xFFFF) : g_xn_zero_page;
      asm volatile("global_load_dwordx4 %0, %1, off" : "=v"(pr[j]) : "v"(p) : "memory");
    }
  };
  auto patch_wait = [&](int stores_since) __attribute__((always_inline)) {
    if (!ASM_LOADS) return;
    constexpr int FULL = MT * NT, FULL_POOL = MT * NT * 3 / 2;
    if (stores_since == FULL) __builtin_amdgcn_s_waitcnt(0x0F70 | (FULL & 15) | ((FULL >> 4) << 14));
    else if (stores_since == FULL_POOL) __builtin_amdgcn_s_waitcnt(0x0F70 | (FULL_POOL & 15) | ((FULL_POOL >> 4) << 14));
    else __builtin_amdgcn_s_waitcnt(0x0F70);
#pragma unroll
    for (int j = 0; j < G::PJ; ++j) asm volatile("" : "+v"(pr[j]));
  };
  auto store_patch = [&]() __attribute__((always_inline)) {
#pragma unroll
    for (int j = 0; j < G::PJ; ++j) {
      if (pdst[j] < 0) continue;
      if (ASM_LOADS) {
        unsigned h[2], l[2];
        xn_split4(pr[j], xs, h, l);
        *reinterpret_cast<uint2*>(patch_h + pdst[j]) = make_uint2(h[0], h[1]);
        *reinterpret_cast<uint2*>(patch_l + pdst[j]) = make_uint2(l[0], l[1]);
      } else {
        f16x4 h, l;
#pragma unroll
        for (int e = 0; e < 4; ++e) {
          const float v = pr[j][e] * xs;
          h[e] = (_Float16)v;
          l[e] = (_Float16)((v - (float)h[e]) * 2048.0f);
        }
        *reinterpret_cast<f16x4*>(patch_h + pdst[j]) = h;
        *reinterpret_cast<f16x4*>(patch_l + pdst[j]) = l;
      }
    }
  };

  const int fi = lane & 15, fg = lane >> 4;
// ... 41 lines not shown
#pragma unroll
      for (int ni = 0; ni < NT; ++ni) acc[mi][ni] = (f32x4){0.f, 0.f, 0.f, 0.f};
#pragma unroll
    for (int s = 0; s < G::NS; ++s) {
      int toff = 0;
      if (TWO) {
        toff = ((s / KK) * G::PW + (s % KK)) * 16;
      } else {
#pragma unroll
        for (int j = 0; j < G::TPP; ++j) {
          const int t = s * G::TPP + j < G::NTAPS ? s * G::TPP + j : 0;
          const int o = ((t / KK) * G::PW + (t % KK)) * CT;
          toff = (jl == j) ? o : toff;
        }
      }
      asm volatile("" : "+v"(toff));
      f16x8 wh[NT], wl[NT], ws[NT], ph[MT], pl[MT];
      const bool last_half = G::HALF && s == G::NS - 1;
#pragma unroll
      for (int ni = 0; ni < NT; ++ni) {
        int bo = s * G::COUT * 32 + b_rd[ni];
        if (last_half) {
          const int row = ni * 16 + fi;
          bo = s * G::COUT * 32 + row * 16 + 8 * ((fg & 1) ^ (pswz(row) & 1));
        }
        wh[ni] = *reinterpret_cast<const f16x8*>(filt_h + bo);
        wl[ni] = *reinterpret_cast<const f16x8*>(filt_l + bo);
        ws[ni] = wh[ni] * (_Float16)(1.0f / 2048.0f);
      }
#pragma unroll
      for (int mi = 0; mi < MT; ++mi) {
        int ad = a_base[mi] + toff;
        if (!TWO && CT == 32) {
          const int pix = ad >> 5;
          ad = (pix << 5) + 8 * (cgl ^ pswz(pix));
        }
        ph[mi] = *reinterpret_cast<const f16x8*>(patch_h + ad);
        pl[mi] = *reinterpret_cast<const f16x8*>(patch_l + ad);
        if (last_half && jl > 0) {
          ph[mi] = (f16x8){0, 0, 0, 0, 0, 0, 0, 0};
          pl[mi] = (f16x8){0, 0, 0, 0, 0, 0, 0, 0};
        }
      }
#pragma unroll
      for (int mi = 0; mi < MT; ++mi)
#pragma unroll
        for (int ni = 0; ni < NT; ++ni) {
          acc[mi][ni] = __builtin_amdgcn_mfma_f32_16x16x32_f16(wh[ni], ph[mi], acc[mi][ni], 0, 0, 0);
          acc[mi][ni] = __builtin_amdgcn_mfma_f32_16x16x32_f16(ws[ni], pl[mi], acc[mi][ni], 0, 0, 0);
          acc[mi][ni] = __builtin_amdgcn_mfma_f32_16x16x32_f16(wl[ni], ph[mi], acc[mi][ni], 0, 0, 0);
        }
    }

    int pm = tile;
    const int tx = pm % a.tiles_x;
    pm /= a.tiles_x;
    const int ty = pm % a.tiles_y;
    const int img = pm / a.tiles_y;
    const int oh0 = ty * 16, ow0 = tx * 16;
    stores_since = (a.cout_valid == G::COUT && oh0 + wave * MT + MT <= a.H && !a.res && !a.scale) ? (a.yp ? MT * NT * 3 / 2 : MT * NT) : -1;
#pragma unroll
    for (int mi = 0; mi < MT; ++mi) {
      const int oh = oh0 + wave * MT + mi, ow = ow0 + fi;
      if (oh >= a.H || ow >= a.W) continue;
      const size_t pix = ((size_t)img * a.H + oh) * a.W + ow;
#pragma unroll
      for (int ni = 0; ni < NT; ++ni) {
        const int co = ni * 16 + 4 * fg;
        f32x4 v = acc[mi][ni] * inv_s;
        if (a.cout_valid == G::COUT) {
          v += bias_r[ni];
          shdr::act_apply4<(TANH ? 2 : 0)>(v, a.act1);
          if (a.scale) v = v * *reinterpret_cast<const f32x4*>(a.scale + co) + *reinterpret_cast<const f32x4*>(a.shift + co);
          if (a.res) {
#pragma unroll
            for (int e = 0; e < 4; ++e) v[e] += a.res[pix * a.res_cs + co + e];
          }
          shdr::act_apply4<(TANH ? 2 : 0)>(v, a.act2);
          *reinterpret_cast<f32x4*>(a.y + pix * G::COUT + co) = v;
#ifndef SHDR_ABL_NO_YM
          if (a.yr) ym = fmaxf(fmaxf(fmaxf(fmaxf(ym, fabsf(v[0])), fabsf(v[1])), fabsf(v[2])), fabsf(v[3]));
#endif
          acc[mi][ni] = v;
        } else {
          if (co >= a.cout_valid) continue;
          f32x4 t = {0.f, 0.f, 0.f, 0.f};
#pragma unroll
          for (int e = 0; e < 4; ++e)
            if (a.bias && co + e < a.cout_valid) t[e] = a.bias[co + e];
          v += t;
          shdr::act_apply4<(TANH ? 2 : 0)>(v, a.act1);
          const bool three = a.cout_valid == 3;
          if (three && a.res) {
            const f32x3u r3 = *reinterpret_cast<const f32x3u*>(a.res + pix * a.res_cs);
            t = (f32x4){r3.x, r3.y, r3.z, 0.f};
          }
#pragma unroll
          for (int e = 0; e < 4; ++e)
            if (co + e < a.cout_valid) {
              if (a.scale) v[e] = v[e] * a.scale[co + e] + a.shift[co + e];
              if (a.res) v[e] += three ? t[e] : a.res[pix * a.res_cs + co + e];
            }
          shdr::act_apply4<(TANH ? 2 : 0)>(v, a.act2);
          if (three) {
            f32x3u o3;
            o3.x = v[0]; o3.y = v[1]; o3.z = v[2];
            *reinterpret_cast<f32x3u*>(a.y + pix * 3) = o3;
// ... 161 lines not shown
}
extern "C" int shdr_conv2d_x3n_prepare_filter_premax_f32(const shdr_conv2d_desc* d, const float* w, float* prepared, int premax, void* stream) {
  SHDR_REQUIRE(d && w && prepared, SHDR_E_NULL, "conv2d_x3n_prepare_filter: null pointer");
  SHDR_REQUIRE(shdr::aligned16(prepared), SHDR_E_ALIGN, "conv2d_x3n_prepare_filter: prepared must be 16-byte aligned");
  hipStream_t st = reinterpret_cast<hipStream_t>(stream);
  const int ct = ct_of(d), Creal = d->C1 + d->C2, ntaps = d->KH * d->KW, ns = (ntaps * ct + 31) / 32;
  const int cv = d->cout_valid > 0 ? d->cout_valid : d->Cout;
  const long nw = (long)ntaps * Creal * d->Cout;
  if (!premax) {
    if (hipMemsetAsync(prepared, 0, XN_HEADER_FLOATS * sizeof(float), st) != hipSuccess) return shdr::fail(SHDR_E_LAUNCH, "conv2d_x3n_prepare_filter: memset");
    hipLaunchKernelGGL(x3n_absmax_kernel, dim3(shdr::stream_grid(nw) < 64 ? shdr::stream_grid(nw) : 64), dim3(256), 0, st, w, nw,
                       reinterpret_cast<unsigned*>(prepared));
  }
  hipLaunchKernelGGL(x3n_pack_kernel, dim3(shdr::stream_grid((long)ns * d->Cout * 32)), dim3(256), 0, st, w, prepared,
                     reinterpret_cast<_Float16*>(prepared + XN_HEADER_FLOATS), ntaps, ct, d->C1, Creal, cv, d->Cout, d->Cout, ns,
#ifdef SHDR_ABL_X3N_NO_HALF
                     d->C2 > 0 ? d->x2_scale : 1.0f, 0);
#else
                     d->C2 > 0 ? d->x2_scale : 1.0f, (d->C2 == 0 && ct == 16 && ntaps % 2 == 1 && ntaps >= 25) ? 1 : 0);
#endif
  return shdr::check_launch("conv2d_x3n_prepare_filter");
}

extern "C" int shdr_conv2d_fwd_x3n_ranged_f32(const shdr_conv2d_desc* d, const float* x1, const float* x2, const float* prepared, const float* bias,
                                              const float* scale, const float* shift, const float* residual, float* y, float* y_pool,
                                              const float* x1_range, const float* x2_range, float* y_range, void* stream) {
  SHDR_REQUIRE(d && x1 && prepared && y, SHDR_E_NULL, "conv2d_x3n: null desc/x1/filter/y");
  SHDR_REQUIRE(!y_pool || (d->H % 2 == 0 && d->W % 2 == 0 && shdr::aligned16(y_pool) && (d->cout_valid == 0 || d->cout_valid == d->Cout)),
               SHDR_E_SHAPE, "conv2d_x3n: the pooled output needs even H, W and every filter column stored");
  SHDR_REQUIRE(shdr_conv2d_x3n_ok_f32(d), SHDR_E_SHAPE, "conv2d_x3n: layer shape not taken by this kernel");
  SHDR_REQUIRE((d->C2 == 0) == (x2 == nullptr), SHDR_E_NULL, "conv2d_x3n: x2 must be given iff C2 > 0");
  SHDR_REQUIRE((scale == nullptr) == (shift == nullptr), SHDR_E_NULL, "conv2d_x3n: scale and shift come together");
  SHDR_REQUIRE(!residual || d->res_cstride >= (d->cout_valid > 0 ? d->cout_valid : d->Cout), SHDR_E_SHAPE, "conv2d_x3n: res_cstride");
  SHDR_REQUIRE(shdr::aligned16(x1) && (!x2 || shdr::aligned16(x2)) && shdr::aligned16(prepared) && shdr::aligned16(y) && (!bias || shdr::aligned16(bias)),
               SHDR_E_ALIGN, "conv2d_x3n: tensors must be 16-byte aligned");
  X3nArgs a{};
  a.x1 = x1; a.x2 = x2;
  a.hdr = prepared;
  a.wp = reinterpret_cast<const _Float16*>(prepared + XN_HEADER_FLOATS);
  a.bias = bias; a.scale = scale; a.shift = shift; a.res = residual; a.y = y;
  a.yp = y_pool; a.pool_avg = d->pool == SHDR_POOL_AVG;
  a.N = d->N; a.H = d->H; a.W = d->W; a.C1 = d->C1;
  a.tiles_x = (d->W + 15) / 16;
  a.tiles_y = (d->H + 15) / 16;
  a.ntiles = a.N * a.tiles_x * a.tiles_y;
  a.act1 = d->act1; a.act2 = d->act2;
  SHDR_REQUIRE(!x2 || ((x1_range == nullptr) == (x2_range == nullptr)), SHDR_E_NULL, "conv2d_x3n: give the range of both sources or of neither");
  a.xr1 = reinterpret_cast<const unsigned*>(x1_range);
  a.xr2 = reinterpret_cast<const unsigned*>(x2 ? x2_range : nullptr);
  if (!x1_range && d->prologue == SHDR_PROLOGUE_RANGE_SCALE) a.xr1 = reinterpret_cast<const unsigned*>(prepared) + 2;
  a.yr = reinterpret_cast<unsigned*>(y_range);
  a.cout_valid = d->cout_valid > 0 ? d->cout_valid : d->Cout;
  a.res_cs = d->res_cstride;
  hipStream_t st = reinterpret_cast<hipStream_t>(stream);
  if (d->Cout == 64) return launch_x3n<3, 8, 4, false>(a, st);
  if (d->Cout == 16) {
    if (d->KH == 3) return dispatch_ct<3, 1>(a, d, st);
    if (d->KH == 5) return dispatch_ct<5, 1>(a, d, st);
    return dispatch_ct<7, 1>(a, d, st);
  }
  if (d->KH == 3) return dispatch_ct<3, 2>(a, d, st);
  if (d->KH == 5) return dispatch_ct<5, 2>(a, d, st);
  return dispatch_ct<7, 2>(a, d, st);
}

extern "C" int shdr_conv2d_fwd_x3n_f32(const shdr_conv2d_desc* d, const float* x1, const float* x2, const float* prepared, const float* bias,
                                       const float* scale, const float* shift, const float* residual, float* y, float* y_pool, void* stream) {
  return shdr_conv2d_fwd_x3n_ranged_f32(d, x1, x2, prepared, bias, scale, shift, residual, y, y_pool, nullptr, nullptr, nullptr, stream);
}
```

### singlehdr-tf2_amd/csrc/frontend.hip

```cpp
#include <stdlib.h>

#include "shdr_internal.h"

namespace {
typedef float nt4 __attribute__((ext_vector_type(4)));


__device__ __forceinline__ float soft_bin(float x, int i , float two_b, float nb, float thr) {
#pragma clang fp contract(off)
  const float centre = __fdiv_rn((float)(2 * i - 1), two_b);
  const float d = fabsf(__fsub_rn(x, centre));
  return d < thr ? __fsub_rn(1.0f, __fmul_rn(d, nb)) : 0.0f;
}

__global__ __launch_bounds__(256) void soft_hist_scalar_kernel(const float* __restrict__ x,
                                                               float* __restrict__ y, long npix,
                                                               int C, int B, float thr) {
  const int CO = B * C;
  const long total = npix * CO;
  const float two_b = (float)(2 * B), nb = (float)B;
  for (long e = (long)blockIdx.x * 256 + threadIdx.x; e < total; e += (long)gridDim.x * 256) {
    const long p = e / CO;
    const int ch = (int)(e - p * CO);
    const int bin = ch / C, c = ch - bin * C;
// ... 70 lines not shown
  return i < 0 ? -i : (i >= n ? 2 * n - 2 - i : i);
}

__device__ __forceinline__ float frontend_channel(const float* __restrict__ img, long ibase, int h,
                                                  int w, int H, int W, const float* rgb, int ch) {
  if (ch < 3) return rgb[ch];
  if (ch < 9) {
    const int c = (ch - 3) >> 1, dir = (ch - 3) & 1;
    const int hm = reflect(h - 1, H), hp = reflect(h + 1, H);
    const int wm = reflect(w - 1, W), wp = reflect(w + 1, W);
    auto at = [&](int hh, int ww) { return img[(ibase + (long)hh * W + ww) * 3 + c]; };
    if (dir == 0)
      return (at(hp, wm) - at(hm, wm)) + 2.0f * (at(hp, w) - at(hm, w)) + (at(hp, wp) - at(hm, wp));
    return (at(hm, wp) - at(hm, wm)) + 2.0f * (at(h, wp) - at(h, wm)) + (at(hp, wp) - at(hp, wm));
  }
  int idx, B;
  if (ch < 21) { idx = ch - 9; B = 4; }
  else if (ch < 45) { idx = ch - 21; B = 8; }
  else if (ch < 93) { idx = ch - 45; B = 16; }
  else return 0.0f;
  const int bin = idx / 3, c = idx - bin * 3;
  const float centre = (float)(2 * bin + 1) * (0.5f / (float)B);
  const float d = fabsf(__fsub_rn(rgb[c], centre));
  return d < 1.0f / (float)B ? __fsub_rn(1.0f, __fmul_rn(d, (float)B)) : 0.0f;
}

template <int YC>
__global__ __launch_bounds__(256) void lin_frontend_kernel(const float* __restrict__ img,
                                                           float* __restrict__ y, int N, int H, int W) {
  constexpr int QPP = (YC + 3) / 4;
  const int row = blockIdx.y;
  const int h = row % H;
  const long ibase = (long)(row / H) * H * W;
  const int idx = blockIdx.x * 256 + threadIdx.x;
  if (idx >= W * QPP) return;
  const int w = idx / QPP, ch0 = (idx - w * QPP) * 4;
  const long p = ibase + (long)h * W + w;
  const float rgb[3] = {img[p * 3], img[p * 3 + 1], img[p * 3 + 2]};
  float v[4];
#pragma unroll
  for (int k = 0; k < 4; ++k) v[k] = frontend_channel(img, ibase, h, w, H, W, rgb, ch0 + k);
  float* yp = y + p * YC + ch0;
  if ((YC & 3) == 0) {
    *reinterpret_cast<float4*>(yp) = make_float4(v[0], v[1], v[2], v[3]);
  } else {
#pragma unroll
    for (int k = 0; k < 4; ++k)
      if (ch0 + k < YC) yp[k] = v[k];
  }
}

template <int YC>
__global__ __launch_bounds__(256) void lin_frontend_rows_kernel(const float* __restrict__ img, float* __restrict__ y, int N, int H,
                                                                int W) {
  constexpr int PX = 64;
  __shared__ __attribute__((aligned(16))) float tile[PX * 96];
  __shared__ float rgbs[PX * 3];
  const int row = blockIdx.y;
  const int h = row % H;
  const long ibase = (long)(row / H) * H * W;
  const int w0 = blockIdx.x * PX;
  const int tid = threadIdx.x;
  if (tid < PX) {
    const int w = min(w0 + tid, W - 1);
    const long p = ibase + (long)h * W + w;
    const int hm = reflect(h - 1, H), hp = reflect(h + 1, H), wm = reflect(w - 1, W), wp = reflect(w + 1, W);
    float* t = tile + tid * 96;
#pragma unroll
    for (int c = 0; c < 3; ++c) {
      auto at = [&](int hh, int ww) { return img[(ibase + (long)hh * W + ww) * 3 + c]; };
      const float v = img[p * 3 + c];
      t[c] = v;
      rgbs[tid * 3 + c] = v;
      t[3 + 2 * c] = (at(hp, wm) - at(hm, wm)) + 2.0f * (at(hp, w) - at(hm, w)) + (at(hp, wp) - at(hm, wp));
      t[4 + 2 * c] = (at(hm, wp) - at(hm, wm)) + 2.0f * (at(h, wp) - at(h, wm)) + (at(hp, wp) - at(hp, wm));
    }
    t[93] = 0.0f; t[94] = 0.0f; t[95] = 0.0f;
  }
  __syncthreads();
  if (tid < 252) {
    const int g = tid / 84, k = tid - g * 84;
    const int lvl = k < 12 ? 0 : (k < 36 ? 1 : 2);
    const int idx = k - (lvl == 0 ? 0 : (lvl == 1 ? 12 : 36));
    const int B = 4 << lvl;
    const int bin = idx / 3, c = idx - bin * 3;
    const float centre = (float)(2 * bin + 1) * (0.5f / (float)B);
    const float fB = (float)B, w = 1.0f / fB;
#pragma unroll 4
    for (int px = g; px < PX; px += 3) {
      const float d = fabsf(__fsub_rn(rgbs[px * 3 + c], centre));
      tile[px * 96 + 9 + k] = d < w ? __fsub_rn(1.0f, __fmul_rn(d, fB)) : 0.0f;
    }
  }
  __syncthreads();
  const int npx = min(PX, W - w0);
  float* yo = y + (ibase + (long)h * W + w0) * YC;
  if (YC == 96) {
    const int nq = npx * 24;
    for (int q = tid; q < nq; q += 256) __builtin_nontemporal_store(*reinterpret_cast<const nt4*>(tile + 4 * q), reinterpret_cast<nt4*>(yo + 4 * q));
  } else {
    const int n = npx * 93;
    for (int e = tid; e < n; e += 256) yo[e] = tile[(e / 93) * 96 + e % 93];
  }
}

}

namespace {
__global__ __launch_bounds__(256) void soft_hist_bwd_kernel(const float* __restrict__ x, const float* __restrict__ dy, float* __restrict__ dx,
                                                            long n, int C, int B) {
  const float fb = (float)B, inv_b = 1.0f / fb;
  for (long e = (long)blockIdx.x * 256 + threadIdx.x; e < n; e += (long)gridDim.x * 256) {
    const long p = e / C;
    const int c = (int)(e - p * C);
// ... 13 lines not shown
extern "C" int shdr_soft_hist_bwd_f32(const float* x, const float* dy, float* dx, int64_t npix, int C, int B, void* stream) {
  SHDR_REQUIRE(x && dy && dx, SHDR_E_NULL, "soft_hist_bwd: null pointer");
  SHDR_REQUIRE(npix > 0 && C > 0 && B > 0, SHDR_E_SHAPE, "soft_hist_bwd: npix, C, B must be positive");
  hipLaunchKernelGGL(soft_hist_bwd_kernel, dim3(shdr::stream_grid(npix * C)), dim3(256), 0, reinterpret_cast<hipStream_t>(stream), x, dy, dx,
                     (long)npix * C, C, B);
  return shdr::check_launch("soft_hist_bwd");
}

extern "C" int shdr_soft_hist_fwd_f32(const float* x, float* y, int64_t npix, int C, int B,
                                      void* stream) {
  SHDR_REQUIRE(x && y, SHDR_E_NULL, "soft_hist: null pointer");
  SHDR_REQUIRE(npix >= 0 && C > 0 && B > 0 && B <= 4096, SHDR_E_SHAPE, "soft_hist: bad shape");
  if (npix == 0) return SHDR_OK;
  hipStream_t st = reinterpret_cast<hipStream_t>(stream);
  const float thr = (float)(1.0 / (double)B);
  if (((B * C) & 3) == 0 && shdr::aligned16(y)) {
    const int Q = (B * C) >> 2;
    const long total = (long)npix * Q;
    int g = Q, h = 256;
    while (h) { const int r = g % h; g = h; h = r; }
    const long unit = Q / g;
    if (unit <= 64 && SHDR_ENV("SHDR_FRONTEND_QUADS") == nullptr) {
      long grid = shdr::stream_grid(total);
      grid = (grid + unit - 1) / unit * unit;
      hipLaunchKernelGGL(soft_hist_rows_kernel, dim3((unsigned)grid), dim3(256), 0, st, x, y, (long)npix, C, B, thr);
    } else {
      hipLaunchKernelGGL(soft_hist_quad_kernel, dim3(shdr::stream_grid(total)), dim3(256), 0, st, x, y,
                         (long)npix, C, B, thr);
    }
  } else {
    const long total = (long)npix * B * C;
    hipLaunchKernelGGL(soft_hist_scalar_kernel, dim3(shdr::stream_grid(total)), dim3(256), 0, st, x,
                       y, (long)npix, C, B, thr);
  }
  return shdr::check_launch("soft_hist");
}

extern "C" int shdr_lin_frontend_fwd_f32(const float* img, float* y, int N, int H, int W,
                                         int y_channels, void* stream) {
  SHDR_REQUIRE(img && y, SHDR_E_NULL, "lin_frontend: null pointer");
  SHDR_REQUIRE(N > 0 && H >= 2 && W >= 2, SHDR_E_SHAPE, "lin_frontend: need N>0, H,W>=2 (REFLECT pad)");
  SHDR_REQUIRE(y_channels >= 93, SHDR_E_SHAPE, "lin_frontend: y_channels must be >= 93");
  SHDR_REQUIRE((y_channels & 3) != 0 || shdr::aligned16(y), SHDR_E_ALIGN, "lin_frontend: y not 16-byte aligned");
  SHDR_REQUIRE(y_channels == 93 || y_channels == 96, SHDR_E_SHAPE, "lin_frontend: y_channels must be 93 or 96");
  SHDR_REQUIRE((long)N * H <= 65535, SHDR_E_SHAPE, "lin_frontend: N*H must be <= 65535");
  hipStream_t st = reinterpret_cast<hipStream_t>(stream);
  if (SHDR_ENV("SHDR_FRONTEND_QUADS") != nullptr) {
    const dim3 grid((unsigned)((W * 24 + 255) / 256), (unsigned)(N * H));
    if (y_channels == 96) hipLaunchKernelGGL(lin_frontend_kernel<96>, grid, dim3(256), 0, st, img, y, N, H, W);
    else hipLaunchKernelGGL(lin_frontend_kernel<93>, grid, dim3(256), 0, st, img, y, N, H, W);
    return shdr::check_launch("lin_frontend");
  }
  const dim3 grid((unsigned)((W + 63) / 64), (unsigned)(N * H));
  if (y_channels == 96) hipLaunchKernelGGL(lin_frontend_rows_kernel<96>, grid, dim3(256), 0, st, img, y, N, H, W);
  else hipLaunchKernelGGL(lin_frontend_rows_kernel<93>, grid, dim3(256), 0, st, img, y, N, H, W);
  return shdr::check_launch("lin_frontend");
}
```

### singlehdr-tf2_amd/csrc/pool.hip

```cpp
#include "shdr_internal.h"

namespace {

__device__ __forceinline__ float4 ld4(const float* p) { return *reinterpret_cast<const float4*>(p); }
__device__ __forceinline__ void st4(float* p, float4 v) { *reinterpret_cast<float4*>(p) = v; }
__device__ __forceinline__ float4 add4(float4 a, float4 b) { return make_float4(a.x + b.x, a.y + b.y, a.z + b.z, a.w + b.w); }
__device__ __forceinline__ float4 max4(float4 a, float4 b) { return make_float4(fmaxf(a.x, b.x), fmaxf(a.y, b.y), fmaxf(a.z, b.z), fmaxf(a.w, b.w)); }

#define SHDR_DECODE_QUAD(e, Q, Wd, Hd, q, w, h, n)                     \
  int q, w, h;                                                          \
  long n;                                                               \
  if ((unsigned long)(e) <= 0xffffffffUL) {                             \
    unsigned _t = (unsigned)(e);                                        \
    q = (int)(_t % (unsigned)(Q)); _t /= (unsigned)(Q);                 \
    w = (int)(_t % (unsigned)(Wd)); _t /= (unsigned)(Wd);               \
    h = (int)(_t % (unsigned)(Hd)); n = (long)(_t / (unsigned)(Hd));    \
  } else {                                                              \
    long _t = (e);                                                      \
    q = (int)(_t % (Q)); _t /= (Q);                                     \
    w = (int)(_t % (Wd)); _t /= (Wd);                                   \
    h = (int)(_t % (Hd)); n = _t / (Hd);                                \
  }

__global__ __launch_bounds__(256) void avgpool2_kernel(const float* __restrict__ x, float* __restrict__ y,
                                                       int N, int H, int W, int C) {
  const int Ho = H >> 1, Wo = W >> 1, Q = C >> 2;
  const long total = (long)N * Ho * Wo * Q;
  for (long e = (long)blockIdx.x * 256 + threadIdx.x; e < total; e += (long)gridDim.x * 256) {
    SHDR_DECODE_QUAD(e, Q, Wo, Ho, q, ow, oh, n)
    const float* p = x + (((n * H + 2 * oh) * W + 2 * ow) * (long)C + 4 * q);
    float4 s = add4(add4(ld4(p), ld4(p + C)), add4(ld4(p + (long)W * C), ld4(p + (long)W * C + C)));
    st4(y + e * 4, make_float4(s.x * 0.25f, s.y * 0.25f, s.z * 0.25f, s.w * 0.25f));
  }
}

__global__ __launch_bounds__(256) void maxpool2_kernel(const float* __restrict__ x, float* __restrict__ y,
                                                       int N, int H, int W, int C) {
  const int Ho = H >> 1, Wo = W >> 1, Q = C >> 2;
  const long total = (long)N * Ho * Wo * Q;
  for (long e = (long)blockIdx.x * 256 + threadIdx.x; e < total; e += (long)gridDim.x * 256) {
    SHDR_DECODE_QUAD(e, Q, Wo, Ho, q, ow, oh, n)
    const float* p = x + (((n * H + 2 * oh) * W + 2 * ow) * (long)C + 4 * q);
    st4(y + e * 4, max4(max4(ld4(p), ld4(p + C)), max4(ld4(p + (long)W * C), ld4(p + (long)W * C + C))));
  }
}

__global__ __launch_bounds__(256) void maxpool3s2_kernel(const float* __restrict__ x, float* __restrict__ y,
                                                         int N, int H, int W, int C, int Ho, int Wo,
                                                         int pt, int pl) {
  const int Q = C >> 2;
  const long total = (long)N * Ho * Wo * Q;
  for (long e = (long)blockIdx.x * 256 + threadIdx.x; e < total; e += (long)gridDim.x * 256) {
    SHDR_DECODE_QUAD(e, Q, Wo, Ho, q, ow, oh, n)
    const float ninf = -__builtin_huge_valf();
    float4 m = make_float4(ninf, ninf, ninf, ninf);
#pragma unroll
    for (int i = 0; i < 3; ++i) {
      const int ih = 2 * oh - pt + i;
      if ((unsigned)ih >= (unsigned)H) continue;
#pragma unroll
      for (int j = 0; j < 3; ++j) {
        const int iw = 2 * ow - pl + j;
        if ((unsigned)iw >= (unsigned)W) continue;
        m = max4(m, ld4(x + (((n * H + ih) * W + iw) * (long)C + 4 * q)));
      }
    }
    st4(y + e * 4, m);
  }
}

__global__ __launch_bounds__(256) void resize2x_kernel(const float* __restrict__ x, float* __restrict__ y,
                                                       int N, int H, int W, int C) {
  const int Q = C >> 2;
  const long total = (long)N * H * W * Q;
  const long orow = (long)2 * W * C;
  auto vl = [](float4 t, float4 u, float ly) {
    return make_float4(t.x + (u.x - t.x) * ly, t.y + (u.y - t.y) * ly, t.z + (u.z - t.z) * ly, t.w + (u.w - t.w) * ly);
  };
  auto load9 = [&](long e, float4 (&v)[3][3], float*& o) {
    SHDR_DECODE_QUAD(e, Q, W, H, q, w, h, n)
    const int hm = max(h - 1, 0), hp = min(h + 1, H - 1), wm = max(w - 1, 0), wp = min(w + 1, W - 1);
    const float* b = x + (n * H * (long)W) * C + 4 * q;
    const int rows[3] = {hm, h, hp};
#pragma unroll
    for (int r = 0; r < 3; ++r) {
      const float* rp = b + (long)rows[r] * W * C;
      v[r][0] = ld4(rp + (long)wm * C); v[r][1] = ld4(rp + (long)w * C); v[r][2] = ld4(rp + (long)wp * C);
    }
    o = y + ((n * 2 * H + 2 * h) * (long)(2 * W) + 2 * w) * C + 4 * q;
  };
  auto emit = [&](const float4 (&v)[3][3], float* o) {
    float4 lo[3], hi[3];
#pragma unroll
    for (int r = 0; r < 3; ++r) {
      const float4 l = v[r][0], c = v[r][1], rr = v[r][2];
      lo[r] = make_float4(l.x + (c.x - l.x) * 0.75f, l.y + (c.y - l.y) * 0.75f, l.z + (c.z - l.z) * 0.75f, l.w + (c.w - l.w) * 0.75f);
      hi[r] = make_float4(c.x + (rr.x - c.x) * 0.25f, c.y + (rr.y - c.y) * 0.25f, c.z + (rr.z - c.z) * 0.25f, c.w + (rr.w - c.w) * 0.25f);
    }
    st4(o, vl(lo[0], lo[1], 0.75f));
    st4(o + C, vl(hi[0], hi[1], 0.75f));
    st4(o + orow, vl(lo[1], lo[2], 0.25f));
    st4(o + orow + C, vl(hi[1], hi[2], 0.25f));
  };
  const long step = (long)gridDim.x * 256;
  long e = (long)blockIdx.x * 256 + threadIdx.x;
// ... 29 lines not shown
      s1 = add4(s1, ld4(xb + (long)(p + 16) * C));
      s2 = add4(s2, ld4(xb + (long)(p + 32) * C));
      s3 = add4(s3, ld4(xb + (long)(p + 48) * C));
    }
    for (; p < HW; p += 16) s = add4(s, ld4(xb + (long)p * C));
    s = add4(add4(s, s1), add4(s2, s3));
  }
  part[g][q] = s;
  __syncthreads();
  if (g == 0 && c0 < C) {
    float4 t = part[0][q];
#pragma unroll
    for (int i = 1; i < 16; ++i) t = add4(t, part[i][q]);
    const float hw = (float)HW;
    st4(y + n * C + c0, make_float4(t.x / hw, t.y / hw, t.z / hw, t.w / hw));
  }
}

int check_nhwc4(const char* op, const void* x, const void* y, int N, int H, int W, int C) {
  SHDR_REQUIRE(x && y, SHDR_E_NULL, "%s: null pointer", op);
  SHDR_REQUIRE(N > 0 && H > 0 && W > 0 && C > 0, SHDR_E_SHAPE, "%s: non-positive dimension", op);
  SHDR_REQUIRE((C & 3) == 0, SHDR_E_ALIGN, "%s: C=%d must be a multiple of 4", op, C);
  SHDR_REQUIRE(shdr::aligned16(x) && shdr::aligned16(y), SHDR_E_ALIGN, "%s: tensors must be 16-byte aligned", op);
  return SHDR_OK;
}

}

extern "C" int shdr_avgpool2_fwd_f32(const float* x, float* y, int N, int H, int W, int C, void* stream) {
  if (int rc = check_nhwc4("avgpool2", x, y, N, H, W, C)) return rc;
  SHDR_REQUIRE(H >= 2 && W >= 2, SHDR_E_SHAPE, "avgpool2: H, W must be >= 2");
  const long total = (long)N * (H / 2) * (W / 2) * (C / 4);
  hipLaunchKernelGGL(avgpool2_kernel, dim3(shdr::stream_grid(total)), dim3(256), 0,
                     reinterpret_cast<hipStream_t>(stream), x, y, N, H, W, C);
  return shdr::check_launch("avgpool2");
}

extern "C" int shdr_maxpool2_fwd_f32(const float* x, float* y, int N, int H, int W, int C, void* stream) {
  if (int rc = check_nhwc4("maxpool2", x, y, N, H, W, C)) return rc;
  SHDR_REQUIRE((H & 1) == 0 && (W & 1) == 0, SHDR_E_SHAPE, "maxpool2: H=%d, W=%d must be even", H, W);
  const long total = (long)N * (H / 2) * (W / 2) * (C / 4);
  hipLaunchKernelGGL(maxpool2_kernel, dim3(shdr::stream_grid(total)), dim3(256), 0,
                     reinterpret_cast<hipStream_t>(stream), x, y, N, H, W, C);
  return shdr::check_launch("maxpool2");
}

extern "C" int shdr_maxpool3s2_fwd_f32(const float* x, float* y, int N, int H, int W, int C, void* stream) {
  if (int rc = check_nhwc4("maxpool3s2", x, y, N, H, W, C)) return rc;
  int Ho, Wo, pt, pl;
  shdr_same_pad(H, 3, 2, &Ho, &pt);
  shdr_same_pad(W, 3, 2, &Wo, &pl);
  const long total = (long)N * Ho * Wo * (C / 4);
  hipLaunchKernelGGL(maxpool3s2_kernel, dim3(shdr::stream_grid(total)), dim3(256), 0,
                     reinterpret_cast<hipStream_t>(stream), x, y, N, H, W, C, Ho, Wo, pt, pl);
  return shdr::check_launch("maxpool3s2");
}

extern "C" int shdr_resize2x_fwd_f32(const float* x, float* y, int N, int H, int W, int C, void* stream) {
  if (int rc = check_nhwc4("resize2x", x, y, N, H, W, C)) return rc;
  const long total = (long)N * H * W * (C / 4);
  hipLaunchKernelGGL(resize2x_kernel, dim3(shdr::stream_grid(total)), dim3(256), 0,
                     reinterpret_cast<hipStream_t>(stream), x, y, N, H, W, C);
  return shdr::check_launch("resize2x");
}

extern "C" int shdr_gap_fwd_f32(const float* x, float* y, int N, int HW, int C, void* stream) {
  if (int rc = check_nhwc4("gap", x, y, N, HW, 1, C)) return rc;
  hipLaunchKernelGGL(gap_kernel, dim3((C + 63) / 64, N), dim3(256), 0,
                     reinterpret_cast<hipStream_t>(stream), x, y, HW, C);
  return shdr::check_launch("gap");
}
```

### singlehdr-tf2_amd/csrc/shdr_internal.h

```cpp
#pragma once
#include <hip/hip_runtime.h>
#include <stdlib.h>
#include <stdarg.h>
#include <stdint.h>
#include <stdio.h>

#include "shdr.h"

namespace shdr {

void set_error(const char* fmt, ...);

inline int fail(int code, const char* fmt, ...) __attribute__((format(printf, 2, 3)));
inline int fail(int code, const char* fmt, ...) {
  char buf[512];
  va_list ap;
  va_start(ap, fmt);
  vsnprintf(buf, sizeof(buf), fmt, ap);
  va_end(ap);
  set_error("%s", buf);
  return code;
}

inline int check_launch(const char* what) {
  hipError_t e = hipGetLastError();
  if (e != hipSuccess) return fail(SHDR_E_LAUNCH, "%s: %s", what, hipGetErrorString(e));
  return SHDR_OK;
}

constexpr int kMaxDevices = 16;
inline int device_slot() {
  int d = 0;
  if (hipGetDevice(&d) != hipSuccess) d = 0;
  return d & (kMaxDevices - 1);
}

inline bool aligned16(const void* p) { return (reinterpret_cast<uintptr_t>(p) & 15u) == 0; }

extern int g_env_epoch;
struct EnvSlot {
  int epoch = -1;
  const char* value = nullptr;
};
inline const char* env_cached(EnvSlot& slot, const char* name) {
  const int e = __atomic_load_n(&g_env_epoch, __ATOMIC_ACQUIRE);
  if (slot.epoch != e) {
    slot.value = getenv(name);
    slot.epoch = e;
  }
  return slot.value;
}
#define SHDR_ENV(name) ([]() -> const char* { static ::shdr::EnvSlot slot; return ::shdr::env_cached(slot, name); }())

#define SHDR_REQUIRE(cond, code, ...) \
  do {                                \
    if (!(cond)) return ::shdr::fail((code), __VA_ARGS__); \
  } while (0)

template <int N>
class StageTimer {
 public:
  StageTimer(float* out, hipStream_t st) : out_(out), st_(st) {
    if (!out_) return;
    while (made_ <= N && hipEventCreate(&ev_[made_]) == hipSuccess) ++made_;
    mark();
  }
  StageTimer(const StageTimer&) = delete;
  StageTimer& operator=(const StageTimer&) = delete;
  void mark() {
    if (marks_ == recorded_ && recorded_ < made_ && hipEventRecord(ev_[recorded_], st_) == hipSuccess) ++recorded_;
    ++marks_;
  }
  ~StageTimer() {
    if (!out_) return;
    const bool ok = recorded_ > 0 && hipEventSynchronize(ev_[recorded_ - 1]) == hipSuccess;
    for (int i = 0; i < N; ++i) {
      if (i + 1 >= marks_) out_[i] = 0.0f;
      else if (!ok || i + 1 >= recorded_ || hipEventElapsedTime(&out_[i], ev_[i], ev_[i + 1]) != hipSuccess) out_[i] = -1.0f;
    }
    for (int i = 0; i < made_; ++i) (void)hipEventDestroy(ev_[i]);
  }

 private:
  float* out_;
  hipStream_t st_;
  hipEvent_t ev_[N + 1];
  int made_ = 0, marks_ = 0, recorded_ = 0;
};

inline int stream_grid(int64_t work_items, int block = 256) {
  int64_t g = (work_items + block - 1) / block;
  if (g < 1) g = 1;
  if (g > 256 * 8) g = 256 * 8;
  return static_cast<int>(g);
}

template <typename KernelT>
inline long block_slots(KernelT kernel, int threads, size_t lds) {
  int dev = 0, cus = 0, occ = 0;
  if (hipGetDevice(&dev) != hipSuccess || hipDeviceGetAttribute(&cus, hipDeviceAttributeMultiprocessorCount, dev) != hipSuccess ||
      hipOccupancyMaxActiveBlocksPerMultiprocessor(&occ, kernel, threads, lds) != hipSuccess || cus < 1 || occ < 1)
    return 0;
  return (long)cus * occ;
}
inline long slice_for_rounds(long slots, long tiles, long units, long min_slice) {
// ... 110 lines not shown
```

### singlehdr-tf2_amd/csrc/up2_fused.hip

```cpp
#include <hip/hip_fp16.h>
#include <stdlib.h>

#include <type_traits>

#include "shdr_internal.h"

namespace {

using f32x4 = __attribute__((ext_vector_type(4))) float;
using f16x8 = __attribute__((ext_vector_type(8))) _Float16;

inline hipStream_t S(void* s) { return reinterpret_cast<hipStream_t>(s); }

constexpr int UF_HEADER_FLOATS = 16;
constexpr int UF_IMG_HALVES = 64 * 32, UF_UNIT_HALVES = 2 * UF_IMG_HALVES;
constexpr int UF_R = 8;
constexpr int UF_COLS = 14;
constexpr int UF_MAX_CIN = 128;
constexpr int UF_THREADS = 256;
constexpr int uf_stride(int CMAX) { return CMAX == 32 ? 32 : CMAX + 8; }

struct UpFusedArgs {
  const float* x;
  const _Float16* wp;
  const float* hdr;
  const float* bias;
  const float* scale;
  const float* shift;
  const float* proj;
  float* y;
  float* yproj;
  const unsigned* xr;
  unsigned* yr;
  int N, h, w, C1, nty, ntx, act1, act2;
  int npatch;
};

__device__ __forceinline__ void uf_range_scale(const unsigned* r, float& xs, float& ixs) {
  xs = 1.0f;
  ixs = 1.0f;
  const unsigned b = r ? *r : 0u;
  if (b != 0u && b < 0x7f800000u) {
    int ex;
    frexpf(__uint_as_float(b), &ex);
    int T = 11 - ex;
    T = T < -126 ? -126 : (T > 126 ? 126 : T);
    xs = ldexpf(1.0f, T);
    ixs = ldexpf(1.0f, -T);
  }
}
__device__ __forceinline__ void uf_split4(const f32x4 v, float xs, unsigned (&h)[2], unsigned (&l)[2]) {
  const float k2048 = 2048.0f;
#pragma unroll
  for (int p = 0; p < 2; ++p) {
    float t0, t1;
    asm("v_fma_mixlo_f16 %0, %1, %2, 0" : "=v"(h[p]) : "v"(v[2 * p]), "s"(xs));
    asm("v_fma_mixhi_f16 %0, %1, %2, 0" : "+v"(h[p]) : "v"(v[2 * p + 1]), "s"(xs));
    asm("v_fma_mix_f32 %0, %1, %2, -%3 op_sel_hi:[0,0,1]" : "=v"(t0) : "v"(v[2 * p]), "s"(xs), "v"(h[p]));
    asm("v_fma_mix_f32 %0, %1, %2, -%3 op_sel:[0,0,1] op_sel_hi:[0,0,1]" : "=v"(t1) : "v"(v[2 * p + 1]), "s"(xs), "v"(h[p]));
    asm("v_fma_mixlo_f16 %0, %1, %2, 0" : "=v"(l[p]) : "v"(t0), "s"(k2048));
    asm("v_fma_mixhi_f16 %0, %1, %2, 0" : "+v"(l[p]) : "v"(t1), "s"(k2048));
  }
}

__device__ __forceinline__ f32x4 mul4(f32x4 a, float s) {
  f32x4 r;
#pragma unroll
  for (int e = 0; e < 4; ++e) r[e] = __fmul_rn(a[e], s);
  return r;
}
__device__ __forceinline__ f32x4 fma4(f32x4 a, float s, f32x4 c) {
  f32x4 r;
#pragma unroll
  for (int e = 0; e < 4; ++e) r[e] = __builtin_fmaf(a[e], s, c[e]);
  return r;
}
__device__ __forceinline__ f32x4 fma4v(f32x4 a, f32x4 s, f32x4 c) {
  f32x4 r;
#pragma unroll
  for (int e = 0; e < 4; ++e) r[e] = __builtin_fmaf(a[e], s[e], c[e]);
  return r;
}
__device__ __forceinline__ f32x4 from_left(f32x4 a) {
  f32x4 r;
#pragma unroll
  for (int e = 0; e < 4; ++e) r[e] = __int_as_float(__builtin_amdgcn_update_dpp(0, __float_as_int(a[e]), 0x111, 0xf, 0xf, true));
  return r;
}
__device__ __forceinline__ f32x4 from_right(f32x4 a) {
  f32x4 r;
#pragma unroll
  for (int e = 0; e < 4; ++e) r[e] = __int_as_float(__builtin_amdgcn_update_dpp(0, __float_as_int(a[e]), 0x101, 0xf, 0xf, true));
  return r;
}

__device__ __forceinline__ int uf_xcd_remap(int bid, int nwg) {
  const int q = nwg >> 3, r = nwg & 7, xcd = bid & 7, idx = bid >> 3;
  return (xcd < r ? xcd * (q + 1) : r * (q + 1) + (xcd - r) * q) + idx;
}

template <int R, int CW, int CMAX>
__global__ __launch_bounds__(UF_THREADS, 2) void up2_fused_kernel(const UpFusedArgs a) {
  constexpr int UF_STRIDE = uf_stride(CMAX);
  constexpr int COUT = 16 * CW, PPB = 4 / CW, GT = 64 * CW;
  constexpr int NPIX = 16 * R, IMG = NPIX * UF_STRIDE;
  constexpr int RO = R - 2;
  extern __shared__ __attribute__((aligned(16))) _Float16 fsm_all[];

  const int lane = threadIdx.x & 63;
  const int wave = __builtin_amdgcn_readfirstlane(threadIdx.x >> 6);
  const int ps = PPB == 1 ? 0 : wave / CW;
  const int cw = PPB == 1 ? wave : wave % CW;
  const int tid = PPB == 1 ? threadIdx.x : threadIdx.x & (GT - 1);
  _Float16* const fsm = fsm_all + ps * (2 * IMG);
  const float* const projp = CW == 4 ? a.proj : nullptr;
  int L = uf_xcd_remap(blockIdx.x, gridDim.x) * PPB + ps;
  const bool patch_ok = PPB == 1 || L < a.npatch;
  if (!patch_ok) L = 0;
  const int tx_ = L % a.ntx; L /= a.ntx;
  const int ty_ = L % a.nty;
  const int n = L / a.nty;
  const int m_start = ty_ * RO, j_start = tx_ * UF_COLS;
  const int nch = a.C1 >> 5;

  float xs, ixs;
  {
    const int f4n = a.C1 >> 2, total = NPIX * f4n;
    const float* xb = a.x + (size_t)n * a.h * a.w * a.C1;
    uf_range_scale(a.xr, xs, ixs);
#pragma unroll 1
    for (int id0 = patch_ok ? tid : total; id0 < total; id0 += 4 * GT) {
      f32x4 v[4];
      int dst[4];
#pragma unroll
      for (int k = 0; k < 4; ++k) {
        const int id = id0 + k * GT;
        dst[k] = -1;
        if (id < total) {
          const int pp = id / f4n, f = id - pp * f4n;
          const int row = min(max(m_start - 1 + (pp >> 4), 0), a.h - 1), col = min(max(j_start - 1 + (pp & 15), 0), a.w - 1);
          v[k] = *reinterpret_cast<const f32x4*>(xb + ((size_t)row * a.w + col) * a.C1 + 4 * f);
          dst[k] = pp * UF_STRIDE + 4 * f;
        }
      }
#pragma unroll
      for (int k = 0; k < 4; ++k) {
        if (dst[k] >= 0) {
          unsigned h[2], l[2];
          uf_split4(v[k], xs, h, l);
          *reinterpret_cast<uint2*>(fsm + dst[k]) = make_uint2(h[0], h[1]);
          *reinterpret_cast<uint2*>(fsm + IMG + dst[k]) = make_uint2(l[0], l[1]);
        }
      }
    }
  }
  __syncthreads();

  const int p = lane & 15, fg = lane >> 4;
  const int j0 = j_start - 1 + p;
  const bool lane_ok = p >= 1 && p <= UF_COLS && j0 < a.w;
  const float wl0 = j0 >= 1 ? 0.75f : 0.0f, wl1 = j0 >= 1 ? 0.25f : 0.0f;
  const float wr0 = j0 + 1 < a.w ? 0.25f : 0.0f, wr1 = j0 + 1 < a.w ? 0.75f : 0.0f;
  const float inv_s = a.hdr[1] * ixs;
  const _Float16* wlane = a.wp + p * 32 + 8 * fg;
  const _Float16* xlane = fsm + p * UF_STRIDE + 8 * fg;

  f32x4 out[RO][2][2];

  auto pass = [&](auto tyc) __attribute__((always_inline)) {
// ... 206 lines not shown
  const bool narrow = uf_narrow_shape_ok(d) && shdr_conv2d_up2_narrow_enabled();
  if (!(uf_shape_ok(d) || narrow) || SHDR_ENV("SHDR_NO_UP2_FUSED") != nullptr || SHDR_ENV("SHDR_NO_UP2_LOWRES") != nullptr ||
      SHDR_ENV("SHDR_NO_WINOGRAD") != nullptr || SHDR_ENV("SHDR_NO_X3") != nullptr)
    return 0;
  if (d->algo != SHDR_ALGO_AUTO || d->prologue != SHDR_PROLOGUE_BILINEAR2X) return 0;
  if ((d->cout_valid != 0 && d->cout_valid != d->Cout) || d->w_batch_stride != 0 || d->y_pix_stride > 1 || (d->y_cstride != 0 && d->y_cstride != d->Cout)) return 0;
  if (d->act1 == SHDR_ACT_TANH || d->act2 == SHDR_ACT_TANH) return 0;
  const long nblk = (long)d->N * ((d->H / 2 + UF_R - 3) / (UF_R - 2)) * ((d->W / 2 + UF_COLS - 1) / UF_COLS);
  return nblk <= 0x7fffffffL - (narrow ? 4 : 0) ? 1 : 0;
}

extern "C" int64_t shdr_conv2d_up2_fused_filter_elems_f32(const shdr_conv2d_desc* d) {
  if (uf_shape_ok(d)) return shdr_conv2d_up2_lowres_filter_elems_f32(d);
  shdr_conv2d_desc g;
  if (!uf_narrow_gemm_desc(d, &g)) return -1;
  const int64_t packed = shdr_conv2d_x3_filter_elems_f32(&g);
  return packed < 0 ? -1 : packed + (int64_t)g.C1 * g.Cout;
}
extern "C" int shdr_conv2d_up2_fused_prepare_filter_f32(const shdr_conv2d_desc* d, const float* w, float* prepared, void* stream) {
  if (uf_shape_ok(d)) return shdr_conv2d_up2_lowres_prepare_filter_f32(d, w, prepared, stream);
  SHDR_REQUIRE(d && w && prepared, SHDR_E_NULL, "up2_fused_prepare_filter: null pointer");
  shdr_conv2d_desc g;
  SHDR_REQUIRE(uf_narrow_gemm_desc(d, &g), SHDR_E_SHAPE,
               "up2_fused_prepare_filter: need a 3x3 layer with one source, even H and W, and Cin 64 / 96 / 128 -> 64, Cin 32 .. 128 -> 32 or Cin 32 / 64 -> 16");
  const int64_t packed = shdr_conv2d_x3_filter_elems_f32(&g);
  SHDR_REQUIRE(packed > 0, SHDR_E_SHAPE, "up2_fused_prepare_filter: the 1x1 form of this layer has no packed filter");
  float* staged = prepared + packed;
  const long total = (long)g.C1 * g.Cout;
  hipLaunchKernelGGL(up2_fused_filter_kernel, dim3(shdr::stream_grid(total)), dim3(256), 0, S(stream), w, staged, g.C1, d->Cout, g.Cout);
  if (int rc = shdr::check_launch("up2_fused_filter")) return rc;
  return shdr_conv2d_x3_prepare_filter_f32(&g, staged, prepared, stream);
}

extern "C" int shdr_conv2d_fwd_up2_fused_f32(const shdr_conv2d_desc* d, const float* x, const float* prepared, const float* bias, const float* scale,
                                             const float* shift, const float* proj, float* y_proj, float* y, const float* x_range, float* y_range,
                                             void* stream) {
  SHDR_REQUIRE(d && x && prepared && x_range, SHDR_E_NULL, "conv2d_up2_fused: null desc / x / prepared filter / x_range");
  SHDR_REQUIRE(y || y_proj, SHDR_E_NULL, "conv2d_up2_fused: neither y nor y_proj");
  SHDR_REQUIRE((proj == nullptr) == (y_proj == nullptr), SHDR_E_NULL, "conv2d_up2_fused: proj and y_proj come together");
  SHDR_REQUIRE(shdr_conv2d_up2_fused_ok_f32(d), SHDR_E_SHAPE, "conv2d_up2_fused: layer not taken (shdr_conv2d_up2_fused_ok_f32)");
  SHDR_REQUIRE(!proj || d->Cout == 64, SHDR_E_SHAPE, "conv2d_up2_fused: the projected output is the 64-cout form's");
  SHDR_REQUIRE((scale == nullptr) == (shift == nullptr), SHDR_E_NULL, "conv2d_up2_fused: scale and shift come together");
  SHDR_REQUIRE(shdr::aligned16(x) && shdr::aligned16(prepared) && (!y || shdr::aligned16(y)) && (!bias || shdr::aligned16(bias)) &&
                   (!scale || (shdr::aligned16(scale) && shdr::aligned16(shift))) && (!proj || shdr::aligned16(proj)),
               SHDR_E_ALIGN, "conv2d_up2_fused: tensors must be 16-byte aligned");
  UpFusedArgs a{};
  a.x = x; a.hdr = prepared; a.wp = reinterpret_cast<const _Float16*>(prepared + UF_HEADER_FLOATS);
  a.bias = bias; a.scale = scale; a.shift = shift; a.proj = proj; a.y = y; a.yproj = y_proj;
  a.xr = reinterpret_cast<const unsigned*>(x_range); a.yr = reinterpret_cast<unsigned*>(y_range);
  a.N = d->N; a.h = d->H / 2; a.w = d->W / 2; a.C1 = d->C1; a.act1 = d->act1; a.act2 = d->act2;
  a.nty = (a.h + UF_R - 3) / (UF_R - 2);
  a.ntx = (a.w + UF_COLS - 1) / UF_COLS;
  a.npatch = (int)((long)a.N * a.nty * a.ntx);
  hipStream_t st = S(stream);
  if (d->Cout == 64) return uf_launch<4, 128>(a, st);
  if (d->Cout == 32) return d->C1 <= 64 ? uf_launch<2, 64>(a, st) : uf_launch<2, 128>(a, st);
  return d->C1 <= 32 ? uf_launch<1, 32>(a, st) : uf_launch<1, 64>(a, st);
}
```

### singlehdr-tf2_amd/csrc/up2_lowres.hip

```cpp
#include <stdlib.h>

#include "shdr_internal.h"

namespace {

typedef float f32x4 __attribute__((ext_vector_type(4)));

inline hipStream_t S(void* s) { return reinterpret_cast<hipStream_t>(s); }
inline size_t up256(size_t b) { return (b + 255) & ~(size_t)255; }
constexpr size_t kRangeScratch = 256;
inline int z_columns(int Cout) {
  const int cols = 9 * Cout, c128 = (cols + 127) / 128 * 128, c256 = (cols + 255) / 256 * 256;
  if (const char* e = SHDR_ENV("SHDR_UP2_LOWRES_PAD")) return atoi(e) == 256 ? c256 : c128;
  return (c256 - cols) * 8 <= cols ? c256 : c128;
}

__global__ __launch_bounds__(256) void up2_lowres_filter_kernel(const float* __restrict__ w, float* __restrict__ st, int Cin, int Cout, int Cp) {
  const long total = (long)Cin * Cp;
  for (long e = (long)blockIdx.x * 256 + threadIdx.x; e < total; e += (long)gridDim.x * 256) {
    const int col = (int)(e % Cp), ci = (int)(e / Cp);
    const int t = col / Cout, co = col - t * Cout;
    st[e] = t < 9 ? w[((size_t)t * Cin + ci) * Cout + co] : 0.0f;
  }
}

constexpr int UL_COLS = 16, UL_QUADS = 16;
struct UpLowArgs {
  const float* z;
  const float* bias;
  const float* scale;
  const float* shift;
  float* y;
  unsigned* yr;
  int N, h, w, Cout, Cp, rows, nseg, nstrip, ncs, act1, act2;
};

__device__ __forceinline__ f32x4 mul4(f32x4 a, float s) {
  f32x4 r;
#pragma unroll
  for (int e = 0; e < 4; ++e) r[e] = __fmul_rn(a[e], s);
  return r;
}
__device__ __forceinline__ f32x4 fma4(f32x4 a, float s, f32x4 c) {
  f32x4 r;
#pragma unroll
  for (int e = 0; e < 4; ++e) r[e] = __builtin_fmaf(a[e], s, c[e]);
  return r;
}
__device__ __forceinline__ f32x4 fma4v(f32x4 a, f32x4 s, f32x4 c) {
  f32x4 r;
#pragma unroll
  for (int e = 0; e < 4; ++e) r[e] = __builtin_fmaf(a[e], s[e], c[e]);
  return r;
}

__device__ __forceinline__ int ul_xcd_remap(int bid, int nwg) {
  const int q = nwg >> 3, r = nwg & 7, xcd = bid & 7, idx = bid >> 3;
  return (xcd < r ? xcd * (q + 1) : r * (q + 1) + (xcd - r) * q) + idx;
}

__global__ __launch_bounds__(256, 2) void up2_lowres_stencil_kernel(const UpLowArgs a) {
  const int tid = threadIdx.x;
  int L = ul_xcd_remap(blockIdx.x, gridDim.x);
  const int cs = L % a.ncs; L /= a.ncs;
  const int strip = L % a.nstrip; L /= a.nstrip;
  const int seg = L % a.nseg;
  const int n = L / a.nseg;
  const int c = cs * (4 * UL_QUADS) + 4 * (tid & (UL_QUADS - 1));
  const int j0 = strip * UL_COLS + (tid >> 4);
  const bool active = j0 < a.w;
  const int m_begin = seg * a.rows, m_end = min(m_begin + a.rows, a.h);
  float ym = 0.0f;
  if (active) {
    const int jm = max(j0 - 1, 0), jp = min(j0 + 1, a.w - 1);
    const float wl0 = j0 >= 1 ? 0.75f : 0.0f, wl1 = j0 >= 1 ? 0.25f : 0.0f;
    const float wr0 = j0 + 1 < a.w ? 0.25f : 0.0f, wr1 = j0 + 1 < a.w ? 0.75f : 0.0f;
    const float* zb = a.z + (size_t)n * a.h * a.w * a.Cp + c;
    const int C = a.Cout;
    auto ld = [](const float* p) __attribute__((always_inline)) { return *reinterpret_cast<const f32x4*>(p); };
    auto hrow = [&](int m, f32x4 (&H)[3][2]) __attribute__((always_inline)) {
      const float* zr = zb + (size_t)m * a.w * a.Cp;
      const float* pm = zr + (size_t)jm * a.Cp;
      const float* p0 = zr + (size_t)j0 * a.Cp;
      const float* pp = zr + (size_t)jp * a.Cp;
      f32x4 v[3][7];
#pragma unroll
      for (int ty = 0; ty < 3; ++ty) {
        const int t0 = 3 * ty * C;
        v[ty][0] = ld(pm + t0); v[ty][1] = ld(p0 + t0);
        v[ty][2] = ld(pm + t0 + C); v[ty][3] = ld(p0 + t0 + C); v[ty][4] = ld(pp + t0 + C);
        v[ty][5] = ld(p0 + t0 + 2 * C); v[ty][6] = ld(pp + t0 + 2 * C);
      }
#pragma unroll
      for (int ty = 0; ty < 3; ++ty) {
        f32x4 t = mul4(v[ty][0], wl0);
        t = fma4(v[ty][1], wl1, t);
        t = fma4(v[ty][2], 0.25f, t);
        t = fma4(v[ty][3], 0.75f, t);
        t = fma4(v[ty][5], 0.75f, t);
        t = fma4(v[ty][6], 0.25f, t);
        H[ty][0] = t;
        f32x4 u = mul4(v[ty][0], 0.25f);
        u = fma4(v[ty][1], 0.75f, u);
        u = fma4(v[ty][3], 0.75f, u);
        u = fma4(v[ty][4], 0.25f, u);
        u = fma4(v[ty][5], wr0, u);
        u = fma4(v[ty][6], wr1, u);
        H[ty][1] = u;
      }
    };
    const f32x4 bias_r = a.bias ? ld(a.bias + c) : (f32x4){0.f, 0.f, 0.f, 0.f};
    const f32x4 scale_r = a.scale ? ld(a.scale + c) : (f32x4){1.f, 1.f, 1.f, 1.f};
    const f32x4 shift_r = a.scale ? ld(a.shift + c) : (f32x4){0.f, 0.f, 0.f, 0.f};
    float* yb = a.y + ((size_t)n * 2 * a.h * 2 * a.w + 2 * j0) * C + c;
    auto finish = [&](f32x4 v, int r, int s) __attribute__((always_inline)) {
      v += bias_r;
      shdr::act_apply4<0>(v, a.act1);
      if (a.scale) v = fma4v(v, scale_r, shift_r);
      shdr::act_apply4<0>(v, a.act2);
      *reinterpret_cast<f32x4*>(yb + ((size_t)r * 2 * a.w + s) * C) = v;
      ym = fmaxf(fmaxf(fmaxf(fmaxf(ym, fabsf(v[0])), fabsf(v[1])), fabsf(v[2])), fabsf(v[3]));
    };
    auto emit = [&](int m0, const f32x4 (&P)[3][2], const f32x4 (&Q)[3][2], const f32x4 (&R)[3][2]) __attribute__((always_inline)) {
      const float wt0 = m0 >= 1 ? 0.75f : 0.0f, wt1 = m0 >= 1 ? 0.25f : 0.0f;
      const float wb0 = m0 + 1 < a.h ? 0.25f : 0.0f, wb1 = m0 + 1 < a.h ? 0.75f : 0.0f;
#pragma unroll
      for (int s = 0; s < 2; ++s) {
        f32x4 t = mul4(P[0][s], wt0);
        t = fma4(Q[0][s], wt1, t);
        t = fma4(P[1][s], 0.25f, t);
        t = fma4(Q[1][s], 0.75f, t);
        t = fma4(Q[2][s], 0.75f, t);
        t = fma4(R[2][s], 0.25f, t);
        finish(t, 2 * m0, s);
        f32x4 u = mul4(P[0][s], 0.25f);
        u = fma4(Q[0][s], 0.75f, u);
        u = fma4(Q[1][s], 0.75f, u);
        u = fma4(R[1][s], 0.25f, u);
        u = fma4(Q[2][s], wb0, u);
        u = fma4(R[2][s], wb1, u);
        finish(u, 2 * m0 + 1, s);
      }
    };
    f32x4 Hw[3][3][2];
    hrow(max(m_begin - 1, 0), Hw[0]);
    hrow(m_begin, Hw[1]);
#pragma unroll 1
    for (int m0 = m_begin; m0 < m_end; m0 += 3) {
#pragma unroll
      for (int u = 0; u < 3; ++u) {
        if (m0 + u < m_end) {
          hrow(min(m0 + u + 1, a.h - 1), Hw[(u + 2) % 3]);
          emit(m0 + u, Hw[u % 3], Hw[(u + 1) % 3], Hw[(u + 2) % 3]);
        }
      }
    }
  }
  if (a.yr) shdr::range_out_block256(a.yr, ym);
}

bool gemm_desc(const shdr_conv2d_desc* d, shdr_conv2d_desc* g) {
  if (!d || d->Cout <= 0 || d->H <= 0 || d->W <= 0 || d->H % 2 || d->W % 2) return false;
  *g = shdr_conv2d_desc{};
  g->N = d->N; g->H = d->H / 2; g->W = d->W / 2; g->C1 = d->C1; g->C2 = 0;
  g->Cout = z_columns(d->Cout);
  g->KH = 1; g->KW = 1; g->stride = 1; g->pad_t = 0; g->pad_l = 0; g->Ho = g->H; g->Wo = g->W;
  g->x2_scale = 1.0f; g->act1 = SHDR_ACT_NONE; g->act2 = SHDR_ACT_NONE; g->algo = SHDR_ALGO_AUTO; g->cout_valid = g->Cout; g->y_cstride = g->Cout;
  return true;
}

}

extern "C" int shdr_conv2d_up2_lowres_ok_f32(const shdr_conv2d_desc* d) {
  shdr_conv2d_desc g;
  if (!gemm_desc(d, &g) || SHDR_ENV("SHDR_NO_UP2_LOWRES") != nullptr || SHDR_ENV("SHDR_NO_WINOGRAD") != nullptr) return 0;
  if (d->algo != SHDR_ALGO_AUTO || d->prologue != SHDR_PROLOGUE_BILINEAR2X || d->KH != 3 || d->KW != 3 || d->stride != 1 || d->pad_t != 1 || d->pad_l != 1 ||
      d->Ho != d->H || d->Wo != d->W || d->C2 != 0 || d->C1 % 32 || d->C1 < 64 || d->Cout % 64)
    return 0;
  if ((d->cout_valid != 0 && d->cout_valid != d->Cout) || d->w_batch_stride != 0 || d->y_pix_stride > 1 || (d->y_cstride != 0 && d->y_cstride != d->Cout)) return 0;
  if (d->act1 == SHDR_ACT_TANH || d->act2 == SHDR_ACT_TANH) return 0;
  if ((long)g.N * g.H * g.W >= (1L << 30)) return 0;
  return shdr_conv2d_x3_ok_f32(&g);
}

extern "C" int64_t shdr_conv2d_up2_lowres_filter_elems_f32(const shdr_conv2d_desc* d) {
  shdr_conv2d_desc g;
  if (!gemm_desc(d, &g) || d->C1 <= 0 || d->C1 % 32 || d->Cout % 64) return -1;
  const int64_t packed = shdr_conv2d_x3_filter_elems_f32(&g);
  return packed < 0 ? -1 : packed + (int64_t)g.C1 * g.Cout;
}

extern "C" int shdr_conv2d_up2_lowres_prepare_filter_f32(const shdr_conv2d_desc* d, const float* w, float* prepared, void* stream) {
  SHDR_REQUIRE(d && w && prepared, SHDR_E_NULL, "up2_lowres_prepare_filter: null pointer");
  shdr_conv2d_desc g;
  SHDR_REQUIRE(gemm_desc(d, &g) && d->KH == 3 && d->KW == 3 && d->C2 == 0 && d->C1 > 0 && d->C1 % 32 == 0 && d->Cout % 64 == 0, SHDR_E_SHAPE,
               "up2_lowres_prepare_filter: need a 3x3 layer with one source, Cin %% 32 == 0, Cout %% 64 == 0, even H and W");
  const int64_t packed = shdr_conv2d_x3_filter_elems_f32(&g);
  SHDR_REQUIRE(packed > 0, SHDR_E_SHAPE, "up2_lowres_prepare_filter: the 1x1 form of this layer has no packed filter");
  float* staged = prepared + packed;
  const long total = (long)g.C1 * g.Cout;
  hipLaunchKernelGGL(up2_lowres_filter_kernel, dim3(shdr::stream_grid(total)), dim3(256), 0, S(stream), w, staged, g.C1, d->Cout, g.Cout);
  if (int rc = shdr::check_launch("up2_lowres_filter")) return rc;
  return shdr_conv2d_x3_prepare_filter_f32(&g, staged, prepared, stream);
}

extern "C" int64_t shdr_conv2d_up2_lowres_workspace_bytes_f32(const shdr_conv2d_desc* d) {
  shdr_conv2d_desc g;
  if (!gemm_desc(d, &g)) return -1;
  return (int64_t)(up256((size_t)g.N * g.H * g.W * g.Cout * sizeof(float)) + kRangeScratch);
}

extern "C" int shdr_conv2d_fwd_up2_lowres_f32(const shdr_conv2d_desc* d, const float* x, const float* prepared, const float* bias, const float* scale,
                                              const float* shift, float* y, void* workspace, const float* x_range, float* y_range, void* stream) {
  SHDR_REQUIRE(d && x && prepared && y && workspace, SHDR_E_NULL, "conv2d_up2_lowres: null desc / x / prepared filter / y / workspace");
  SHDR_REQUIRE(shdr_conv2d_up2_lowres_ok_f32(d), SHDR_E_SHAPE, "conv2d_up2_lowres: layer not taken (shdr_conv2d_up2_lowres_ok_f32)");
  SHDR_REQUIRE((scale == nullptr) == (shift == nullptr), SHDR_E_NULL, "conv2d_up2_lowres: scale and shift come together");
  SHDR_REQUIRE(shdr::aligned16(x) && shdr::aligned16(prepared) && shdr::aligned16(workspace) && shdr::aligned16(y) && (!bias || shdr::aligned16(bias)) && (!scale || (shdr::aligned16(scale) && shdr::aligned16(shift))),
               SHDR_E_ALIGN, "conv2d_up2_lowres: tensors must be 16-byte aligned");
  shdr_conv2d_desc g;
  gemm_desc(d, &g);
  float* z = reinterpret_cast<float*>(workspace);
  if (!x_range) {
    float* slot = reinterpret_cast<float*>(reinterpret_cast<char*>(workspace) + shdr_conv2d_up2_lowres_workspace_bytes_f32(d) - kRangeScratch);
    if (hipMemsetAsync(slot, 0, sizeof(float), S(stream)) != hipSuccess) return shdr::fail(SHDR_E_LAUNCH, "conv2d_up2_lowres: memset failed");
    if (int rc = shdr_absmax_f32(x, (int64_t)g.N * g.H * g.W * g.C1, slot, stream)) return rc;
    x_range = slot;
  }
  if (int rc = shdr_conv2d_fwd_x3_ranged_f32(&g, x, nullptr, prepared, nullptr, nullptr, nullptr, z, nullptr, x_range, nullptr, nullptr, stream)) return rc;
  UpLowArgs a{};
  a.z = z; a.bias = bias; a.scale = scale; a.shift = shift; a.y = y; a.yr = reinterpret_cast<unsigned*>(y_range);
  a.N = g.N; a.h = g.H; a.w = g.W; a.Cout = d->Cout; a.Cp = g.Cout; a.act1 = d->act1; a.act2 = d->act2;
  a.nstrip = (a.w + UL_COLS - 1) / UL_COLS;
  a.ncs = a.Cout / (4 * UL_QUADS);
  a.rows = 16;
  while (a.rows > 4 && (long)a.N * ((a.h + a.rows - 1) / a.rows) * a.nstrip * a.ncs < 1024) a.rows >>= 1;
  if (const char* e = SHDR_ENV("SHDR_UP2_LOWRES_ROWS")) a.rows = atoi(e) > 0 ? atoi(e) : a.rows;
  a.nseg = (a.h + a.rows - 1) / a.rows;
  const long nblk = (long)a.N * a.nseg * a.nstrip * a.ncs;
  if (nblk > 0x7fffffffL) return shdr::fail(SHDR_E_SHAPE, "conv2d_up2_lowres: grid of %ld blocks", nblk);
  hipLaunchKernelGGL(up2_lowres_stencil_kernel, dim3((unsigned)nblk), dim3(256), 0, S(stream), a);
  return shdr::check_launch("up2_lowres_stencil_kernel");
}
```

Measured before the change: 968.6.

## Alternate kernel block traversal order and add banded up2 lowres path

Adds a pointer-keyed table that records the block traversal direction used to write each buffer. The next kernel reading that buffer walks its tiles in reverse, so it starts with the data most recently written and likely still in cache. This applies to the conv_x3, conv_x3n, frontend, maxpool, up2_fused and up2_lowres kernels. It also adds a banded up2_lowres entry point that could split the 1x1 GEMM plus stencil into image or row bands to keep the intermediate small. The band size defaults to 0 MB, so the banded path runs as a single band, the same as before. The costs are a mutex-guarded table lookup on every launch and a possible loss of DRAM locality from reversed block order.

```diff
diff --git a/include/shdr.h b/include/shdr.h
--- a/include/shdr.h
+++ b/include/shdr.h
@@ -8,6 +8,10 @@
 #endif
 
 void shdr_config_reload(void);
+
+int shdr_block_order_last(void);
+int shdr_block_order_of(const void* p);
+void shdr_block_order_reset(void);
 
 #define SHDR_OK          0
 #define SHDR_E_SHAPE    (-1)
@@ -103,6 +107,11 @@
 int shdr_conv2d_fwd_up2_lowres_f32(const shdr_conv2d_desc* d, const float* x, const float* prepared, const float* bias,
                                    const float* scale, const float* shift, float* y, void* workspace, const float* x_range,
                                    float* y_range, void* stream);
+
+int64_t shdr_conv2d_up2_lowres_banded_workspace_bytes_f32(const shdr_conv2d_desc* d);
+int shdr_conv2d_fwd_up2_lowres_banded_f32(const shdr_conv2d_desc* d, const float* x, const float* prepared, const float* bias,
+                                          const float* scale, const float* shift, float* y, void* workspace, const float* x_range,
+                                          float* y_range, void* stream);
 
 int shdr_conv2d_up2_fused_ok_f32(const shdr_conv2d_desc* d);
 int shdr_conv2d_up2_narrow_enabled(void);
diff --git a/singlehdr-tf2_amd/_lib.py b/singlehdr-tf2_amd/_lib.py
--- a/singlehdr-tf2_amd/_lib.py
+++ b/singlehdr-tf2_amd/_lib.py
@@ -85,6 +85,9 @@
     "shdr_conv2d_wgrad_x3_ok_f32": (c_int, [ctypes.POINTER(ConvDesc), c_int]),
     "shdr_conv2d_wgrad_x3_f32": (c_int, [ctypes.POINTER(ConvDesc), c_ptr, c_ptr, c_int, c_ptr, c_ptr, c_ptr, c_ptr, c_ptr, c_ptr]),
     "shdr_config_reload": (None, []),
+    "shdr_block_order_last": (c_int, []),
+    "shdr_block_order_of": (c_int, [c_ptr]),
+    "shdr_block_order_reset": (None, []),
     "shdr_conv2d_x3_input_absmax_f32": (c_int, [c_ptr, c_i64, c_ptr, c_ptr]),
     "shdr_conv2d_x3n_ok_f32": (c_int, [ctypes.POINTER(ConvDesc)]),
     "shdr_conv2d_x3n_filter_elems_f32": (c_i64, [ctypes.POINTER(ConvDesc)]),
@@ -112,7 +115,9 @@
     "shdr_conv2d_up2_lowres_prepare_filter_f32": (c_int, [ctypes.POINTER(ConvDesc), c_ptr, c_ptr, c_ptr]),
     "shdr_conv2d_up2_lowres_workspace_bytes_f32": (c_i64, [ctypes.POINTER(ConvDesc)]),
     "shdr_conv2d_fwd_up2_lowres_f32": (c_int, [ctypes.POINTER(ConvDesc)] + [c_ptr] * 10),
-    "shdr_conv2d_up2_fused_ok_f32": (c_int, [ctypes.POINTER(ConvDesc)]),
+    "shdr_conv2d_up2_lowres_banded_workspace_bytes_f32": (c_i64, [ctypes.POINTER(ConvDesc)]),
+    "shdr_conv2d_fwd_up2_lowres_banded_f32": (c_int, [ctypes.POINTER(ConvDesc)] + [c_ptr] * 10),
+    "shdr_conv2d_up2_fused_ok_f32":(c_int, [ctypes.POINTER(ConvDesc)]),
     "shdr_conv2d_up2_narrow_enabled": (c_int, []),
     "shdr_conv2d_up2_fused_filter_elems_f32": (c_i64, [ctypes.POINTER(ConvDesc)]),
     "shdr_conv2d_up2_fused_prepare_filter_f32": (c_int, [ctypes.POINTER(ConvDesc), c_ptr, c_ptr, c_ptr]),
diff --git a/singlehdr-tf2_amd/_ops.py b/singlehdr-tf2_amd/_ops.py
--- a/singlehdr-tf2_amd/_ops.py
+++ b/singlehdr-tf2_amd/_ops.py
@@ -1,6 +1,7 @@
 import collections
 import ctypes
 import math
+import os
 
 import numpy as np
 import torch
@@ -286,12 +287,14 @@
     xr = _range_of(x_in)
     if xr is None:
         RANGE_MISSES[(tuple(x.shape), None, tuple(_d(w).shape))] += 1
-    ws = torch.empty(int(lib.shdr_conv2d_up2_lowres_workspace_bytes_f32(ctypes.byref(d))), device=x.device, dtype=torch.uint8)
+    name = "up2_lowres_f32" if os.environ.get("SHDR_NO_UP2_BANDED") else "up2_lowres_banded_f32"
+    nws = getattr(lib, "shdr_conv2d_%s" % name.replace("_f32", "_workspace_bytes_f32"))(ctypes.byref(d))
+    ws = torch.empty(int(nws), device=x.device, dtype=torch.uint8)
     out = torch.empty((d.N, d.H, d.W, d.Cout), device=x.device, dtype=torch.float32)
     yr = _new_slot(x.device)
-    rc = lib.shdr_conv2d_fwd_up2_lowres_f32(ctypes.byref(d), _ptr(x), _ptr(prepared), _ptr(_d(bias)), _ptr(_d(scale)), _ptr(_d(shift)),
-                                            _ptr(out), _ptr(ws), _ptr(xr), _ptr(yr), _stream())
-    _lib.check(rc, "shdr_conv2d_fwd_up2_lowres_f32")
+    rc = getattr(lib, "shdr_conv2d_fwd_" + name)(ctypes.byref(d), _ptr(x), _ptr(prepared), _ptr(_d(bias)), _ptr(_d(scale)), _ptr(_d(shift)),
+                                                 _ptr(out), _ptr(ws), _ptr(xr), _ptr(yr), _stream())
+    _lib.check(rc, "shdr_conv2d_fwd_" + name)
     return _set_range(out, yr)
 
 
diff --git a/singlehdr-tf2_amd/build.py b/singlehdr-tf2_amd/build.py
--- a/singlehdr-tf2_amd/build.py
+++ b/singlehdr-tf2_amd/build.py
@@ -70,7 +70,7 @@
 def build(force=False, verbose=True):
     hipcc = _hipcc()
     os.makedirs(OBJ_DIR, exist_ok=True)
-    headers = [os.path.join(CSRC, "shdr_internal.h"), os.path.join(CSRC, "linear_resize.h"), os.path.join(CSRC, "jpeg_int.h"), os.path.join(CSRC, "deflate_huffman.h"),
+    headers = [os.path.join(CSRC, "shdr_internal.h"), os.path.join(CSRC, "block_order.h"), os.path.join(CSRC, "linear_resize.h"), os.path.join(CSRC, "jpeg_int.h"), os.path.join(CSRC, "deflate_huffman.h"),
                os.path.join(CSRC, "deflate_lz.h"), os.path.join(CSRC, "deflate_batch.h"),
                os.path.join(CSRC, "inflate.h"), os.path.join(CSRC, "piz.h"), os.path.join(CSRC, "jpeg_scan.h"),
                os.path.join(CSRC, "exr_half.h"), os.path.join(INCLUDE, "shdr.h"), __file__]
diff --git a/singlehdr-tf2_amd/csrc/api.cpp b/singlehdr-tf2_amd/csrc/api.cpp
--- a/singlehdr-tf2_amd/csrc/api.cpp
+++ b/singlehdr-tf2_amd/csrc/api.cpp
@@ -19,6 +19,13 @@
 int g_env_epoch = 0;
 }
 extern "C" void shdr_config_reload(void) { __atomic_add_fetch(&shdr::g_env_epoch, 1, __ATOMIC_ACQ_REL); }
+
+extern "C" int shdr_block_order_last(void) { return shdr::block_order_last(); }
+extern "C" int shdr_block_order_of(const void* p) { return shdr::block_order_table().lookup(p); }
+extern "C" void shdr_block_order_reset(void) {
+  shdr::block_order_table().clear();
+  shdr::block_order_last() = -1;
+}
 
 extern "C" const char* shdr_last_error(void) { return shdr::g_last_error; }
 extern "C" const char* shdr_version(void) { return "libshdr 0.1 gfx950"; }
diff --git a/singlehdr-tf2_amd/csrc/block_order.h b/singlehdr-tf2_amd/csrc/block_order.h
--- /dev/null
+++ b/singlehdr-tf2_amd/csrc/block_order.h
@@ -0,0 +1,67 @@
+#pragma once
+#include <stdint.h>
+
+#include <mutex>
+
+namespace shdr {
+
+constexpr int kOrderFwd = 0, kOrderRev = 1;
+
+class BlockOrderTable {
+ public:
+  static constexpr int kEntries = 256;
+
+  int lookup(const void* p) {
+    std::lock_guard<std::mutex> lock(mu_);
+    const int i = find(p);
+    return i < 0 ? -1 : order_[i];
+  }
+  int next(const void* in, const void* const* outs, int nout, int forced = -1) {
+    std::lock_guard<std::mutex> lock(mu_);
+    int order = forced;
+    if (order < 0) {
+      const int i = find(in);
+      order = i < 0 ? kOrderFwd : !order_[i];
+    }
+    for (int k = 0; k < nout; ++k)
+      if (outs[k]) put(outs[k], order);
+    return order;
+  }
+  void clear() {
+    std::lock_guard<std::mutex> lock(mu_);
+    for (int i = 0; i < kEntries; ++i) ptr_[i] = nullptr;
+    cursor_ = 0;
+  }
+
+ private:
+  int find(const void* p) const {
+    if (!p) return -1;
+    for (int i = 0; i < kEntries; ++i)
+      if (ptr_[i] == p) return i;
+    return -1;
+  }
+  void put(const void* p, int order) {
+    int i = find(p);
+    if (i < 0) {
+      i = cursor_;
+      cursor_ = (cursor_ + 1) % kEntries;
+      ptr_[i] = p;
+    }
+    order_[i] = (uint8_t)order;
+  }
+  std::mutex mu_;
+  const void* ptr_[kEntries] = {};
+  uint8_t order_[kEntries] = {};
+  int cursor_ = 0;
+};
+
+inline BlockOrderTable& block_order_table() {
+  static BlockOrderTable table;
+  return table;
+}
+inline int& block_order_last() {
+  static thread_local int last = -1;
+  return last;
+}
+
+}
diff --git a/singlehdr-tf2_amd/csrc/conv_x3.hip b/singlehdr-tf2_amd/csrc/conv_x3.hip
--- a/singlehdr-tf2_amd/csrc/conv_x3.hip
+++ b/singlehdr-tf2_amd/csrc/conv_x3.hip
@@ -53,6 +53,7 @@
   const _Float16* pwp[4];
   const float* proj;
   float* yproj;
+  int rev;
 };
 
 __device__ __forceinline__ void x3_range_scale(const unsigned* r1, const unsigned* r2, float& xs, float& ixs) {
@@ -210,6 +211,10 @@
   const int q = nwg >> 3, r = nwg & 7, xcd = bid & 7, idx = bid >> 3;
   return (xcd < r ? xcd * (q + 1) : r * (q + 1) + (xcd - r) * q) + idx;
 }
+__device__ __forceinline__ int x3_block(const X3Args& a) {
+  const int nblk = a.nblk_m * a.nblk_n, L = xcd_remap(blockIdx.x, nblk);
+  return a.rev ? nblk - 1 - L : L;
+}
 __host__ __device__ inline int f4(int row) { return (-(row >> 2)) & 3; }
 __host__ __device__ inline int sx(int col) { return ((col >> 2) & 1) * 2; }
 __device__ __forceinline__ int pcol(int fi) { return fi < 4 ? fi : (fi >= 12 ? fi - 8 : fi + 4); }
@@ -229,7 +234,7 @@
 
   const int tid = threadIdx.x, lane = tid & 63;
   const int wave = __builtin_amdgcn_readfirstlane(tid >> 6);
-  const int L = xcd_remap(blockIdx.x, a.nblk_m * a.nblk_n);
+  const int L = x3_block(a);
   const int pn = L % a.nblk_n;
   int pm = L / a.nblk_n;
   const int tx = pm % a.tiles_x;
@@ -546,7 +551,7 @@
   const int tid = threadIdx.x, lane = tid & 63;
   const int wave = __builtin_amdgcn_readfirstlane(tid >> 6);
   const int slice = wave % NS, grp = wave / NS;
-  const int L = xcd_remap(blockIdx.x, a.nblk_m * a.nblk_n);
+  const int L = x3_block(a);
   const int pn = L % a.nblk_n, pm = L / a.nblk_n;
   const int P0 = pm * BP, Ptot = a.N * a.H * a.W;
 
@@ -732,7 +737,7 @@
   const int tid = threadIdx.x, lane = tid & 63;
   const int wave = __builtin_amdgcn_readfirstlane(tid >> 6);
   const int slice = wave >> 2, wq = wave & 3;
-  const int L = xcd_remap(blockIdx.x, a.nblk_m * a.nblk_n);
+  const int L = x3_block(a);
   const int pn = L % a.nblk_n;
   int pm = L / a.nblk_n;
   const int tx = pm % a.tiles_x;
@@ -1258,6 +1263,7 @@
   SHDR_REQUIRE(!residual || (d->stride == 1 && d->res_cstride >= d->Cout && d->res_cstride % 4 == 0 && shdr::aligned16(residual) && !y_pool && !proj), SHDR_E_SHAPE,
                "conv2d_x3: the residual takes a stride-1 layer, res_cstride >= Cout (a multiple of 4), a 16-byte aligned tensor, no pooled / projected output");
   a.res = residual; a.res_cs = d->res_cstride;
+  a.rev = shdr::block_order(x1, y, y_pool, y_proj);
   hipStream_t st = reinterpret_cast<hipStream_t>(stream);
   X3Phase ph[4];
   const int n = x3_phases(d, ph);
diff --git a/singlehdr-tf2_amd/csrc/conv_x3n.hip b/singlehdr-tf2_amd/csrc/conv_x3n.hip
--- a/singlehdr-tf2_amd/csrc/conv_x3n.hip
+++ b/singlehdr-tf2_amd/csrc/conv_x3n.hip
@@ -31,6 +31,7 @@
   const unsigned* xr1;
   const unsigned* xr2;
   unsigned* yr;
+  int rev;
 };
 
 __device__ __forceinline__ void xn_range_scale(const unsigned* r1, const unsigned* r2, float& xs, float& ixs) {
@@ -175,7 +176,7 @@
   f32x4 pr[G::PJ];
   constexpr bool ASM_LOADS = !(CT == 8 && NT == 1);
   auto load_patch = [&](int tile) __attribute__((always_inline)) {
-    int pm = tile;
+    int pm = a.rev ? a.ntiles - 1 - tile : tile;
     const int tx = pm % a.tiles_x;
     pm /= a.tiles_x;
     const int ty = pm % a.tiles_y;
@@ -323,7 +324,7 @@
         }
     }
 
-    int pm = tile;
+    int pm = a.rev ? a.ntiles - 1 - tile : tile;
     const int tx = pm % a.tiles_x;
     pm /= a.tiles_x;
     const int ty = pm % a.tiles_y;
@@ -591,6 +592,7 @@
   a.yr = reinterpret_cast<unsigned*>(y_range);
   a.cout_valid = d->cout_valid > 0 ? d->cout_valid : d->Cout;
   a.res_cs = d->res_cstride;
+  a.rev = shdr::block_order(x1, y, y_pool);
   hipStream_t st = reinterpret_cast<hipStream_t>(stream);
   if (d->Cout == 64) return launch_x3n<3, 8, 4, false>(a, st);
   if (d->Cout == 16) {
diff --git a/singlehdr-tf2_amd/csrc/frontend.hip b/singlehdr-tf2_amd/csrc/frontend.hip
--- a/singlehdr-tf2_amd/csrc/frontend.hip
+++ b/singlehdr-tf2_amd/csrc/frontend.hip
@@ -146,14 +146,14 @@
 
 template <int YC>
 __global__ __launch_bounds__(256) void lin_frontend_rows_kernel(const float* __restrict__ img, float* __restrict__ y, int N, int H,
-                                                                int W) {
+                                                                int W, int rev) {
   constexpr int PX = 64;
   __shared__ __attribute__((aligned(16))) float tile[PX * 96];
   __shared__ float rgbs[PX * 3];
-  const int row = blockIdx.y;
+  const int row = rev ? gridDim.y - 1 - blockIdx.y : blockIdx.y;
   const int h = row % H;
   const long ibase = (long)(row / H) * H * W;
-  const int w0 = blockIdx.x * PX;
+  const int w0 = (rev ? gridDim.x - 1 - blockIdx.x : blockIdx.x) * PX;
   const int tid = threadIdx.x;
   if (tid < PX) {
     const int w = min(w0 + tid, W - 1);
@@ -273,7 +273,8 @@
     return shdr::check_launch("lin_frontend");
   }
   const dim3 grid((unsigned)((W + 63) / 64), (unsigned)(N * H));
-  if (y_channels == 96) hipLaunchKernelGGL(lin_frontend_rows_kernel<96>, grid, dim3(256), 0, st, img, y, N, H, W);
-  else hipLaunchKernelGGL(lin_frontend_rows_kernel<93>, grid, dim3(256), 0, st, img, y, N, H, W);
+  const int rev = shdr::block_order(img, y);
+  if (y_channels == 96) hipLaunchKernelGGL(lin_frontend_rows_kernel<96>, grid, dim3(256), 0, st, img, y, N, H, W, rev);
+  else hipLaunchKernelGGL(lin_frontend_rows_kernel<93>, grid, dim3(256), 0, st, img, y, N, H, W, rev);
   return shdr::check_launch("lin_frontend");
 }
diff --git a/singlehdr-tf2_amd/csrc/pool.hip b/singlehdr-tf2_amd/csrc/pool.hip
--- a/singlehdr-tf2_amd/csrc/pool.hip
+++ b/singlehdr-tf2_amd/csrc/pool.hip
@@ -47,10 +47,11 @@
 
 __global__ __launch_bounds__(256) void maxpool3s2_kernel(const float* __restrict__ x, float* __restrict__ y,
                                                          int N, int H, int W, int C, int Ho, int Wo,
-                                                         int pt, int pl) {
+                                                         int pt, int pl, int rev) {
   const int Q = C >> 2;
   const long total = (long)N * Ho * Wo * Q;
-  for (long e = (long)blockIdx.x * 256 + threadIdx.x; e < total; e += (long)gridDim.x * 256) {
+  for (long i = (long)blockIdx.x * 256 + threadIdx.x; i < total; i += (long)gridDim.x * 256) {
+    const long e = rev ? total - 1 - i : i;
     SHDR_DECODE_QUAD(e, Q, Wo, Ho, q, ow, oh, n)
     const float ninf = -__builtin_huge_valf();
     float4 m = make_float4(ninf, ninf, ninf, ninf);
@@ -186,7 +187,7 @@
   shdr_same_pad(W, 3, 2, &Wo, &pl);
   const long total = (long)N * Ho * Wo * (C / 4);
   hipLaunchKernelGGL(maxpool3s2_kernel, dim3(shdr::stream_grid(total)), dim3(256), 0,
-                     reinterpret_cast<hipStream_t>(stream), x, y, N, H, W, C, Ho, Wo, pt, pl);
+                     reinterpret_cast<hipStream_t>(stream), x, y, N, H, W, C, Ho, Wo, pt, pl, shdr::block_order(x, y));
   return shdr::check_launch("maxpool3s2");
 }
 
diff --git a/singlehdr-tf2_amd/csrc/shdr_internal.h b/singlehdr-tf2_amd/csrc/shdr_internal.h
--- a/singlehdr-tf2_amd/csrc/shdr_internal.h
+++ b/singlehdr-tf2_amd/csrc/shdr_internal.h
@@ -6,6 +6,7 @@
 #include <stdio.h>
 
 #include "shdr.h"
+#include "block_order.h"
 
 namespace shdr {
 
@@ -51,6 +52,13 @@
   return slot.value;
 }
 #define SHDR_ENV(name) ([]() -> const char* { static ::shdr::EnvSlot slot; return ::shdr::env_cached(slot, name); }())
+
+inline int block_order(const void* in, const void* o0, const void* o1 = nullptr, const void* o2 = nullptr) {
+  int forced = -1;
+  if (const char* e = SHDR_ENV("SHDR_BLOCK_ORDER")) forced = e[0] == 'f' ? kOrderFwd : (e[0] == 'r' ? kOrderRev : -1);
+  const void* const outs[3] = {o0, o1, o2};
+  return block_order_last() = block_order_table().next(in, outs, 3, forced);
+}
 
 #define SHDR_REQUIRE(cond, code, ...) \
   do {                                \
diff --git a/singlehdr-tf2_amd/csrc/up2_fused.hip b/singlehdr-tf2_amd/csrc/up2_fused.hip
--- a/singlehdr-tf2_amd/csrc/up2_fused.hip
+++ b/singlehdr-tf2_amd/csrc/up2_fused.hip
@@ -34,6 +34,7 @@
   unsigned* yr;
   int N, h, w, C1, nty, ntx, act1, act2;
   int npatch;
+  int rev;
 };
 
 __device__ __forceinline__ void uf_range_scale(const unsigned* r, float& xs, float& ixs) {
@@ -114,7 +115,8 @@
   const int tid = PPB == 1 ? threadIdx.x : threadIdx.x & (GT - 1);
   _Float16* const fsm = fsm_all + ps * (2 * IMG);
   const float* const projp = CW == 4 ? a.proj : nullptr;
-  int L = uf_xcd_remap(blockIdx.x, gridDim.x) * PPB + ps;
+  const int blk = uf_xcd_remap(blockIdx.x, gridDim.x);
+  int L = (a.rev ? (int)gridDim.x - 1 - blk : blk) * PPB + ps;
   const bool patch_ok = PPB == 1 || L < a.npatch;
   if (!patch_ok) L = 0;
   const int tx_ = L % a.ntx; L /= a.ntx;
@@ -427,6 +429,7 @@
   a.nty = (a.h + UF_R - 3) / (UF_R - 2);
   a.ntx = (a.w + UF_COLS - 1) / UF_COLS;
   a.npatch = (int)((long)a.N * a.nty * a.ntx);
+  a.rev = shdr::block_order(x, y, y_proj);
   hipStream_t st = S(stream);
   if (d->Cout == 64) return uf_launch<4, 128>(a, st);
   if (d->Cout == 32) return d->C1 <= 64 ? uf_launch<2, 64>(a, st) : uf_launch<2, 128>(a, st);
diff --git a/singlehdr-tf2_amd/csrc/up2_lowres.hip b/singlehdr-tf2_amd/csrc/up2_lowres.hip
--- a/singlehdr-tf2_amd/csrc/up2_lowres.hip
+++ b/singlehdr-tf2_amd/csrc/up2_lowres.hip
@@ -33,6 +33,8 @@
   float* y;
   unsigned* yr;
   int N, h, w, Cout, Cp, rows, nseg, nstrip, ncs, act1, act2;
+  int rev;
+  int zh, zrow0, mlo, mhi, img0;
 };
 
 __device__ __forceinline__ f32x4 mul4(f32x4 a, float s) {
@@ -62,6 +64,7 @@
 __global__ __launch_bounds__(256, 2) void up2_lowres_stencil_kernel(const UpLowArgs a) {
   const int tid = threadIdx.x;
   int L = ul_xcd_remap(blockIdx.x, gridDim.x);
+  if (a.rev) L = (int)gridDim.x - 1 - L;
   const int cs = L % a.ncs; L /= a.ncs;
   const int strip = L % a.nstrip; L /= a.nstrip;
   const int seg = L % a.nseg;
@@ -69,17 +72,17 @@
   const int c = cs * (4 * UL_QUADS) + 4 * (tid & (UL_QUADS - 1));
   const int j0 = strip * UL_COLS + (tid >> 4);
   const bool active = j0 < a.w;
-  const int m_begin = seg * a.rows, m_end = min(m_begin + a.rows, a.h);
+  const int m_begin = a.mlo + seg * a.rows, m_end = min(m_begin + a.rows, a.mhi);
   float ym = 0.0f;
   if (active) {
     const int jm = max(j0 - 1, 0), jp = min(j0 + 1, a.w - 1);
     const float wl0 = j0 >= 1 ? 0.75f : 0.0f, wl1 = j0 >= 1 ? 0.25f : 0.0f;
     const float wr0 = j0 + 1 < a.w ? 0.25f : 0.0f, wr1 = j0 + 1 < a.w ? 0.75f : 0.0f;
-    const float* zb = a.z + (size_t)n * a.h * a.w * a.Cp + c;
+    const float* zb = a.z + (size_t)n * a.zh * a.w * a.Cp + c;
     const int C = a.Cout;
     auto ld = [](const float* p) __attribute__((always_inline)) { return *reinterpret_cast<const f32x4*>(p); };
     auto hrow = [&](int m, f32x4 (&H)[3][2]) __attribute__((always_inline)) {
-      const float* zr = zb + (size_t)m * a.w * a.Cp;
+      const float* zr = zb + (size_t)(m - a.zrow0) * a.w * a.Cp;
       const float* pm = zr + (size_t)jm * a.Cp;
       const float* p0 = zr + (size_t)j0 * a.Cp;
       const float* pp = zr + (size_t)jp * a.Cp;
@@ -112,7 +115,7 @@
     const f32x4 bias_r = a.bias ? ld(a.bias + c) : (f32x4){0.f, 0.f, 0.f, 0.f};
     const f32x4 scale_r = a.scale ? ld(a.scale + c) : (f32x4){1.f, 1.f, 1.f, 1.f};
     const f32x4 shift_r = a.scale ? ld(a.shift + c) : (f32x4){0.f, 0.f, 0.f, 0.f};
-    float* yb = a.y + ((size_t)n * 2 * a.h * 2 * a.w + 2 * j0) * C + c;
+    float* yb = a.y + ((size_t)(n + a.img0) * 2 * a.h * 2 * a.w + 2 * j0) * C + c;
     auto finish = [&](f32x4 v, int r, int s) __attribute__((always_inline)) {
       v += bias_r;
       shdr::act_apply4<0>(v, a.act1);
@@ -159,6 +162,21 @@
   if (a.yr) shdr::range_out_block256(a.yr, ym);
 }
 
+int launch_stencil(UpLowArgs& a, hipStream_t st) {
+  const int nrow = a.mhi - a.mlo;
+  a.nstrip = (a.w + UL_COLS - 1) / UL_COLS;
+  a.ncs = a.Cout / (4 * UL_QUADS);
+  a.rows = 16;
+  while (a.rows > 4 && (long)a.N * ((nrow + a.rows - 1) / a.rows) * a.nstrip * a.ncs < 1024) a.rows >>= 1;
+  if (const char* e = SHDR_ENV("SHDR_UP2_LOWRES_ROWS")) a.rows = atoi(e) > 0 ? atoi(e) : a.rows;
+  a.nseg = (nrow + a.rows - 1) / a.rows;
+  const long nblk = (long)a.N * a.nseg * a.nstrip * a.ncs;
+  if (nblk > 0x7fffffffL) return shdr::fail(SHDR_E_SHAPE, "conv2d_up2_lowres: grid of %ld blocks", nblk);
+  a.rev = shdr::block_order(a.z, a.y);
+  hipLaunchKernelGGL(up2_lowres_stencil_kernel, dim3((unsigned)nblk), dim3(256), 0, st, a);
+  return shdr::check_launch("up2_lowres_stencil_kernel");
+}
+
 bool gemm_desc(const shdr_conv2d_desc* d, shdr_conv2d_desc* g) {
   if (!d || d->Cout <= 0 || d->H <= 0 || d->W <= 0 || d->H % 2 || d->W % 2) return false;
   *g = shdr_conv2d_desc{};
@@ -230,14 +248,119 @@
   UpLowArgs a{};
   a.z = z; a.bias = bias; a.scale = scale; a.shift = shift; a.y = y; a.yr = reinterpret_cast<unsigned*>(y_range);
   a.N = g.N; a.h = g.H; a.w = g.W; a.Cout = d->Cout; a.Cp = g.Cout; a.act1 = d->act1; a.act2 = d->act2;
-  a.nstrip = (a.w + UL_COLS - 1) / UL_COLS;
-  a.ncs = a.Cout / (4 * UL_QUADS);
-  a.rows = 16;
-  while (a.rows > 4 && (long)a.N * ((a.h + a.rows - 1) / a.rows) * a.nstrip * a.ncs < 1024) a.rows >>= 1;
-  if (const char* e = SHDR_ENV("SHDR_UP2_LOWRES_ROWS")) a.rows = atoi(e) > 0 ? atoi(e) : a.rows;
-  a.nseg = (a.h + a.rows - 1) / a.rows;
-  const long nblk = (long)a.N * a.nseg * a.nstrip * a.ncs;
-  if (nblk > 0x7fffffffL) return shdr::fail(SHDR_E_SHAPE, "conv2d_up2_lowres: grid of %ld blocks", nblk);
-  hipLaunchKernelGGL(up2_lowres_stencil_kernel, dim3((unsigned)nblk), dim3(256), 0, S(stream), a);
-  return shdr::check_launch("up2_lowres_stencil_kernel");
-}
+  a.zh = a.h; a.zrow0 = 0; a.mlo = 0; a.mhi = a.h; a.img0 = 0;
+  return launch_stencil(a, S(stream));
+}
+
+namespace {
+
+constexpr long kBandSlots = 512;
+constexpr double kBandDefaultMB = 0.0;
+
+struct BandPlan {
+  int imgs;
+  int rows;
+  long pixels;
+};
+
+BandPlan band_plan(const shdr_conv2d_desc& g) {
+  const long img = (long)g.H * g.W, all = (long)g.N * img, bpp = (long)g.Cout * (long)sizeof(float);
+  const BandPlan one{g.N, 0, all};
+  double mb = kBandDefaultMB;
+  if (const char* e = SHDR_ENV("SHDR_UP2_BAND_MB")) mb = atof(e);
+  if (SHDR_ENV("SHDR_NO_UP2_BANDED") != nullptr || !(mb > 0.0)) return one;
+  const long pixels = mb * 1048576.0 / (double)bpp >= (double)all ? all : (long)(mb * 1048576.0 / (double)bpp);
+  if (pixels >= all) return one;
+  BandPlan p = one;
+  if (pixels >= img) {
+    p.imgs = (int)(pixels / img);
+    p.pixels = p.imgs * img;
+  } else {
+    long rows = pixels / g.W - 2;
+    if (rows < 1) rows = 1;
+    const long nblk_n = g.Cout / (g.Cout % 256 == 0 ? 256 : 128), gb = ((rows + 2) * g.W + 127) / 128 * nblk_n;
+    if (gb >= kBandSlots) {
+      const long r2 = (gb / kBandSlots) * kBandSlots / nblk_n * 128 / g.W - 2;
+      if (r2 >= 1 && r2 < rows) rows = r2;
+    }
+    if (rows >= g.H) {
+      p.imgs = 1;
+      p.pixels = img;
+    } else {
+      p.imgs = 0;
+      p.rows = (int)rows;
+      p.pixels = (rows + 2 < g.H ? rows + 2 : g.H) * g.W;
+    }
+  }
+  shdr_conv2d_desc b = g;
+  if (p.imgs > 0) {
+    b.N = p.imgs;
+    bool ok = shdr_conv2d_x3_ok_f32(&b) != 0;
+    if (ok && g.N % p.imgs) {
+      b.N = g.N % p.imgs;
+      ok = shdr_conv2d_x3_ok_f32(&b) != 0;
+    }
+    return ok ? p : one;
+  }
+  b.N = 1;
+  for (int m0 = 0; m0 < g.H; m0 += p.rows) {
+    const int lo = m0 > 0 ? m0 - 1 : 0, hi = m0 + p.rows + 1 < g.H ? m0 + p.rows + 1 : g.H;
+    b.H = b.Ho = hi - lo;
+    if (!shdr_conv2d_x3_ok_f32(&b)) return one;
+  }
+  return p;
+}
+
+}
+
+extern "C" int64_t shdr_conv2d_up2_lowres_banded_workspace_bytes_f32(const shdr_conv2d_desc* d) {
+  shdr_conv2d_desc g;
+  if (!gemm_desc(d, &g)) return -1;
+  return (int64_t)(up256((size_t)band_plan(g).pixels * g.Cout * sizeof(float)) + kRangeScratch);
+}
+
+extern "C" int shdr_conv2d_fwd_up2_lowres_banded_f32(const shdr_conv2d_desc* d, const float* x, const float* prepared, const float* bias,
+                                                     const float* scale, const float* shift, float* y, void* workspace, const float* x_range,
+                                                     float* y_range, void* stream) {
+  SHDR_REQUIRE(d && x && prepared && y && workspace, SHDR_E_NULL, "conv2d_up2_lowres: null desc / x / prepared filter / y / workspace");
+  SHDR_REQUIRE(shdr_conv2d_up2_lowres_ok_f32(d), SHDR_E_SHAPE, "conv2d_up2_lowres: layer not taken (shdr_conv2d_up2_lowres_ok_f32)");
+  SHDR_REQUIRE((scale == nullptr) == (shift == nullptr), SHDR_E_NULL, "conv2d_up2_lowres: scale and shift come together");
+  SHDR_REQUIRE(shdr::aligned16(x) && shdr::aligned16(prepared) && shdr::aligned16(workspace) && shdr::aligned16(y) && (!bias || shdr::aligned16(bias)) && (!scale || (shdr::aligned16(scale) && shdr::aligned16(shift))),
+               SHDR_E_ALIGN, "conv2d_up2_lowres: tensors must be 16-byte aligned");
+  shdr_conv2d_desc g;
+  gemm_desc(d, &g);
+  const BandPlan p = band_plan(g);
+  float* z = reinterpret_cast<float*>(workspace);
+  if (!x_range) {
+    float* slot = reinterpret_cast<float*>(reinterpret_cast<char*>(workspace) + up256((size_t)p.pixels * g.Cout * sizeof(float)));
+    if (hipMemsetAsync(slot, 0, sizeof(float), S(stream)) != hipSuccess) return shdr::fail(SHDR_E_LAUNCH, "conv2d_up2_lowres: memset failed");
+    if (int rc = shdr_absmax_f32(x, (int64_t)g.N * g.H * g.W * g.C1, slot, stream)) return rc;
+    x_range = slot;
+  }
+  UpLowArgs a{};
+  a.z = z; a.bias = bias; a.scale = scale; a.shift = shift; a.y = y; a.yr = reinterpret_cast<unsigned*>(y_range);
+  a.h = g.H; a.w = g.W; a.Cout = d->Cout; a.Cp = g.Cout; a.act1 = d->act1; a.act2 = d->act2;
+  shdr_conv2d_desc b = g;
+  const size_t xrow = (size_t)g.W * g.C1;
+  if (p.imgs > 0) {
+    for (int n0 = 0; n0 < g.N; n0 += p.imgs) {
+      b.N = g.N - n0 < p.imgs ? g.N - n0 : p.imgs;
+      if (int rc = shdr_conv2d_fwd_x3_ranged_f32(&b, x + (size_t)n0 * g.H * xrow, nullptr, prepared, nullptr, nullptr, nullptr, z, nullptr, x_range, nullptr, nullptr, stream)) return rc;
+      a.N = b.N; a.zh = g.H; a.zrow0 = 0; a.mlo = 0; a.mhi = g.H; a.img0 = n0;
+      if (int rc = launch_stencil(a, S(stream))) return rc;
+    }
+    return SHDR_OK;
+  }
+  b.N = 1;
+  for (int n = 0; n < g.N; ++n) {
+    for (int m0 = 0; m0 < g.H; m0 += p.rows) {
+      const int m1 = m0 + p.rows < g.H ? m0 + p.rows : g.H;
+      const int lo = m0 > 0 ? m0 - 1 : 0, hi = m1 < g.H ? m1 + 1 : g.H;
+      b.H = b.Ho = hi - lo;
+      if (int rc = shdr_conv2d_fwd_x3_ranged_f32(&b, x + ((size_t)n * g.H + lo) * xrow, nullptr, prepared, nullptr, nullptr, nullptr, z, nullptr, x_range, nullptr, nullptr, stream)) return rc;
+      a.N = 1; a.zh = hi - lo; a.zrow0 = lo; a.mlo = m0; a.mhi = m1; a.img0 = n;
+      if (int rc = launch_stencil(a, S(stream))) return rc;
+    }
+  }
+  return SHDR_OK;
+}
```

Result: slower. 954.0 (-1.5%).
